# noamzilo/sed-crnn

Hardware: AMD Instinct MI355X
Metric: mel-frames/sec training throughput (seq=256, mel=40) (higher is better)
Workload: dtype f32; 1 GPU; BASELINE config 2: mono (B=128,256,40,1) per GPU, 3xConv3x3(128)+BN+ReLU+pool(1,2)+dropout0.5, BiGRU 2x128, Linear(256,1), BCEWithLogits, Adam lr 1e-3; full fit step (fwd+loss+bwd+allreduce+Adam); global_batch=128, seq_len=256, n_mels=40, parallelism=single

## Files before the change

### include/sedcrnn.h

```cpp
#ifndef SEDCRNN_H
#define SEDCRNN_H

#include <stddef.h>
#include <stdint.h>

#ifdef __cplusplus
extern "C" {
#endif

#define SED_MAX_CONV 4
#define SED_MAX_GRU 4
#define SED_MAX_DENSE 4

int sed_version(void);
const char* sed_last_error_string(void);

int sed_conv3x3_pack_weights(const float* w_oihw, float* wp_fwd, float* wp_dgrad,
                             int Cout, int Cin, void* stream);

int sed_conv3x3_stat_rows(int B, int Cin, int F, int T, int Cout, int x_is_nchw);

int sed_conv3x3_fwd(const float* x, int x_is_nchw, const float* wp, const float* bias,
                    float* y, float* stat_partials,
                    int B, int Cin, int F, int T, int Cout, void* stream);

int sed_conv3x3_pack_weights_ex(const float* w_oihw, float* wp_fwd, float* wp_dgrad, int Cout, int Cin, int mode, void* stream);
int sed_conv3x3_fwd_ex(const float* x, int x_is_nchw, const float* wp, const float* bias, float* y, float* stat_partials,
                       int B, int Cin, int F, int T, int Cout, int mode, void* stream);

size_t sed_conv3x3_wgrad_workspace_bytes(int B, int Cin, int F, int T, int Cout);
int sed_conv3x3_wgrad(const float* x, int x_is_nchw, const float* dy, float* dw_oihw,
                      void* workspace, int B, int Cin, int F, int T, int Cout, void* stream);

#define SED_WGRAD_ZERO_ROW_CLEAN 0x100
#define SED_WGRAD_DIRECT 0x200
size_t sed_conv3x3_wgrad_zero_row_bytes(int B, int Cin, int F, int T, int Cout);
int sed_conv3x3_wgrad_ex(const float* x, int x_is_nchw, const float* dy, float* dw_oihw,
                         void* workspace, int B, int Cin, int F, int T, int Cout, int mode, void* stream);

int sed_conv3x3_bn_relu_pool_eval_supported(int B, int Cin, int F, int T, int Cout);
int sed_conv3x3_pack_weights_bn_folded(const float* w, const float* bias, const float* gamma, const float* beta,
                                       const float* running_mean, const float* running_var, float eps,
                                       float* wf, float* bias_folded, int Cout, int Cin, void* stream);
int sed_conv3x3_bn_relu_pool_eval(const float* x, const float* wp_folded, const float* bias_folded, float* pooled,
                                  int B, int Cin, int F, int T, int Cout, void* stream);
int sed_conv3x3_bf16_eval_supported(int B, int Cin, int F, int T, int Cout);
int sed_conv3x3_bf16_pack_weights_bn_folded(const float* w, const float* bias, const float* gamma, const float* beta,
                                            const float* running_mean, const float* running_var, float eps,
                                            void* wf_bf16, float* bias_folded, int Cout, int Cin, void* stream);
int sed_conv3x3_bf16_bn_relu_pool_eval(const void* x, int x_is_bf16, const void* wf_bf16, const float* bias_folded,
                                       void* pooled_bf16, int B, int Cin, int F, int T, int Cout, void* stream);
int sed_conv3x3_dgrad_bnred_rows(int B, int C, int F, int T, int Cin);
int sed_conv3x3_dgrad_bnred(const float* dy, const float* wp_dgrad, float* dx, float* partials, const float* pooled,
                            const float* gamma, const float* beta, const float* conv_out_below, const float* mean,
                            const float* rstd, float drop_p, int pool_f, int pool_t, int Fy, int Ty,
                            int B, int C, int F, int T, int Cin, void* stream);
int sed_conv3x3_wino_rows(int B, int Cin, int F, int T, int Cout);
int sed_conv3x3_wino_phase_ticks(unsigned long long* buf);
size_t sed_conv3x3_wino_packed_floats(int Cout, int Cin);
int sed_conv3x3_wino_pack_weights(const float* w_oihw, float* uf, float* ud, int Cout, int Cin, void* stream);
int sed_conv3x3_wino_fwd(const float* x, const float* uf, const float* bias, float* y, float* stat_partials,
                         int B, int Cin, int F, int T, int Cout, void* stream);
int sed_conv3x3_wino_dgrad_bnred(const float* dy, const float* ud, float* dx, float* partials, const float* pooled,
                                 const float* gamma, const float* beta, const float* conv_out_below, const float* mean,
                                 const float* rstd, float drop_p, int pool_f, int pool_t, int Fy, int Ty,
                                 int B, int C, int F, int T, int Cin, void* stream);
int sed_conv3x3_wino_pack_weights_bn_folded(const float* w_oihw, const float* bias, const float* gamma, const float* beta,
                                            const float* running_mean, const float* running_var, float eps,
                                            float* uf, float* bias_folded, int Cout, int Cin, void* stream);
int sed_conv3x3_wino_bn_relu_pool_eval(const float* x, const float* uf_folded, const float* bias_folded, float* pooled,
                                       int B, int Cin, int F, int T, int Cout, void* stream);
int sed_conv3x3_wino_rg_rows(int B, int C, int F, int T, int Cin, int Cin1);
int sed_conv3x3_wino_dgrad_bnred_rg(const float* dy, const float* ud, float* dx, float* partials, const float* pooled,
                                    const float* gamma, const float* beta, const float* mean, const float* rstd, float drop_p,
                                    const float* x1, int Cin1, const unsigned char* argmax_bits, float* rg_partials,
                                    int B, int C, int F, int T, int Cin, void* stream);
int sed_conv3x3_dgrad_bnred_rg_rows(int B, int C, int F, int T, int Cin, int Cin1);
int sed_conv3x3_dgrad_bnred_rg(const float* dy, const float* wp_dgrad, float* dx, float* partials, const float* pooled,
                               const float* gamma, const float* beta, const float* mean, const float* rstd, float drop_p,
                               const float* x1, int Cin1, const unsigned char* argmax_bits, float* rg_partials,
                               int B, int C, int F, int T, int Cin, void* stream);

int sed_bn_finalize_train(const float* stat_partials, int rows, int C, double count,
                          const float* gamma, const float* beta,
                          float* running_mean, float* running_var, float momentum, float eps,
                          float* mean, float* rstd, float* scale, float* shift, void* stream);
int sed_bn_stat_sums(const float* stat_partials, int rows, int C, float* sums, void* stream);
int sed_bn_finalize_from_sums(const float* sums, int C, double count, const float* gamma, const float* beta,
                              float* running_mean, float* running_var, float momentum, float eps,
                              float* mean, float* rstd, float* scale, float* shift, void* stream);
int sed_bn_finalize_eval(const float* gamma, const float* beta, const float* running_mean,
                         const float* running_var, float eps, int C,
                         float* scale, float* shift, void* stream);

int sed_bn_relu_pool_drop_fwd(const float* y, const float* scale, const float* shift, float* out,
                              int B, int T, int F, int C, int pool_f, int pool_t, int out_tcf,
                              float drop_p, uint64_t seed, const uint64_t* seed_dev, void* stream);

int sed_bn_relu_pool_route(const float* y, const float* scale, const float* shift, unsigned char* route,
                           int B, int T, int F, int C, int pool_f, int pool_t, void* stream);
int sed_bn_bwd_rows(int B, int T, int pool_t);
int sed_bn_relu_pool_drop_bwd_reduce(const float* y, const float* dout, const float* scale,
                                     const float* shift, const float* mean, const float* rstd,
                                     float* partials, int B, int T, int F, int C, int pool_f,
                                     int pool_t, int out_tcf, float drop_p, uint64_t seed, const uint64_t* seed_dev, void* stream);
int sed_bn_bwd_finalize(const float* partials, int rows, int C, float* sum_g, float* sum_gx,
                        float* dgamma, float* dbeta, void* stream);
int sed_bn_bwd_finalize_small_gamma(const float* partials, int rows, int C, float* sum_g, float* sum_gx,
                                    float* dgamma, float* dbeta, const float* dpooled, const float* pooled,
                                    const float* y, const float* gamma, const float* beta, const float* mean,
                                    const float* rstd, const float* scale, const float* shift,
                                    int B, int T, int F, int pool_f, int pool_t, float drop_p, void* stream);
int sed_bn_bwd_reduce_pooled_supported(int F, int C, int pool_f, int pool_t, int out_tcf);
int sed_bn_bwd_reduce_pooled(const float* pooled, const float* dout, const float* gamma, const float* beta,
                             const float* y, const float* mean, const float* rstd, const float* scale, const float* shift,
                             float* partials, int B, int T, int F, int C, int pool_f, int pool_t, int out_tcf, float drop_p, void* stream);
int sed_bn_relu_pool_drop_bwd_apply(const float* y, const float* dout, const float* scale,
                                    const float* shift, const float* mean, const float* rstd,
                                    const float* sum_g, const float* sum_gx, float* dy,
                                    float* dbias_partials, int B, int T, int F, int C, int pool_f,
                                    int pool_t, int out_tcf, float drop_p, uint64_t seed, const uint64_t* seed_dev, void* stream);
int sed_reduce_rows(const float* partials, int rows, int C, int row_stride, float* out, void* stream);

int sed_conv1_fused_supported(int Cin, int F, int T, int C, int pool_f, int pool_t);
int sed_conv1_fused_rows(int B, int T);
size_t sed_conv1_stats_workspace_bytes(int B, int Cin, int T);
size_t sed_conv1_moments_doubles(int Cin);
int sed_conv1_stats(const float* x, const float* wp, const float* bias, float* stat_partials, void* workspace,
                    int B, int Cin, int F, int T, int C, double* moments, void* stream);
int sed_conv1_bn_relu_pool_drop_fwd(const float* x, const float* wp, const float* bias, const float* scale,
                                    const float* shift, float* out, int B, int Cin, int F, int T, int C,
                                    int pool_f, int pool_t, float drop_p, uint64_t seed, const uint64_t* seed_dev,
                                    unsigned char* argmax_bits, void* stream);
int sed_conv1_route(const float* x, const float* wp, const float* bias, const float* scale, const float* shift,
                    unsigned char* route, int B, int Cin, int F, int T, int C, int pool_f, int pool_t, void* stream);
int sed_conv1_bwd_reduce(const float* x, const float* wp, const float* bias, const float* dout,
                         const float* scale, const float* shift, const float* mean, const float* rstd,
                         float* partials, int B, int Cin, int F, int T, int C, int pool_f, int pool_t,
                         float drop_p, uint64_t seed, const uint64_t* seed_dev, void* stream);
size_t sed_conv1_bwd_apply_workspace_bytes(int B, int Cin, int T, int C);
int sed_conv1_bwd_apply_wgrad(const float* x, const float* wp, const float* bias, const float* dout,
                              const float* scale, const float* shift, const float* mean, const float* rstd,
                              const float* sum_g, const float* sum_gx, float* dw_oihw, float* dbias,
                              void* workspace, int B, int Cin, int F, int T, int C, int pool_f, int pool_t,
                              float drop_p, uint64_t seed, const uint64_t* seed_dev,
                              const float* gamma, const float* beta, float* dgamma, void* stream);

int sed_conv1_rgrad_supported(int Cin, int F, int T, int C, int pool_f, int pool_t);
size_t sed_conv1_bwd_wgrad_workspace_bytes(int B, int Cin, int T, int C);
int sed_conv1_bwd_wgrad(const float* x, const float* dout, const float* pooled, const unsigned char* argmax_bits,
                        const double* moments, const float* wp, const float* bias, const float* mean, const float* rstd,
                        const float* scale, const float* sum_g, const float* sum_gx, float* dw_oihw, float* dbias,
                        void* workspace, int B, int Cin, int F, int T, int C, float drop_p,
                        const float* gamma, const float* beta, float* dgamma, void* stream);
int sed_conv1_bwd_wgrad_assemble(const float* partials, int rows, const double* moments, const float* wp, const float* bias,
                                 const float* mean, const float* rstd, const float* scale, const float* sum_g,
                                 const float* sum_gx, float* dw_oihw, float* dbias, int B, int Cin, int F, int T, int C,
                                 const float* gamma, const float* beta, float* dgamma, void* stream);

int sed_gemm_f32(const float* A, long a_si, long a_sk, const float* B, long b_sk, long b_sj,
                 float* C, long ldc, const float* bias, float beta, int M, int N, int K, void* stream);
size_t sed_gemm_f32_workspace_bytes(int M, int N, int K);
int sed_gemm_f32_ws(const float* A, long a_si, long a_sk, const float* B, long b_sk, long b_sj,
                    float* C, long ldc, const float* bias, int M, int N, int K, void* workspace, void* stream);

int sed_gemm_bf16_nt(const void* A, const void* B, const float* bias, float* C, long ldc, int M, int N, int K, void* stream);

int sed_gemm_f32_wgrad(const float* A, long a_si, long a_sk, const float* B, long b_sk, long b_sj,
                       float* C, long ldc, int M, int N, int K, void* workspace, void* stream);

int sed_linear_fwd(const float* x, const float* W, const float* b, float* y,
                   int M, int K, int N, int relu, void* stream);
size_t sed_linear_bwd_workspace_bytes(int M, int K, int N);
int sed_linear_bwd(const float* x, const float* W, const float* y, float* dy, float* dx,
                   float* dW, float* db, void* workspace, int M, int K, int N, int relu, void* stream);

size_t sed_gru_seq_workspace_bytes(int H);
int sed_gru_seq_fwd(const float* gi, const float* const* whh, const float* const* bhh,
                    float* out, float* saved, void* workspace, int B, int T, int H, void* stream);
size_t sed_gru_seq_bwd_workspace_bytes(int B, int H);
int sed_gru_seq_bwd(const float* dout, const float* saved, const float* const* whh,
                    float* dgi, float* dgh, float* const* dbih, float* const* dbhh, void* workspace,
                    int B, int T, int H, void* stream);
int sed_gru_seq_variant(int B, int H, int* bt, int* hreg, int* hlds);

int sed_loss_fwd_bwd(const float* logits, const float* targets, int n, int kind, float alpha,
                     float gamma, int reduction_mean, float* loss, float* dlogits, float* probs,
                     void* stream);
int sed_sigmoid(const float* x, float* y, int n, void* stream);
int sed_scale(float* x, long n, float alpha, void* stream);

size_t sed_sqnorm_workspace_bytes(long n);
int sed_grad_norm_clip_coef(const float* g, long n, float max_norm, float* norm_out,
                            void* workspace, void* stream);
int sed_adam_step(float* p, const float* g, float* m, float* v, long n, float lr, float beta1,
                  float beta2, float eps, float weight_decay, int step, const float* grad_scale,
                  const uint64_t* step_state, void* stream);
int sed_step_advance(uint64_t* step_state, void* stream);

size_t sed_logmel_tables_bytes(const float* melfb_host, int n_fft, int n_mels);
int sed_logmel_build_tables(const float* window_host, const float* melfb_host, int n_fft, int n_mels,
                            void* tables_host, size_t tables_bytes);
int sed_logmel(const float* pcm, long n_samples, const void* tables, size_t tables_bytes,
               const float* mu, const float* inv_sigma, float* out,
               int n_fft, int hop, int n_mels, int pad_mode, void* stream);
size_t sed_logmel_batch_workspace_bytes(int R);
int sed_logmel_batch(const float* pcm, long pcm_len, const long* clips_host, int R, const void* tables, size_t tables_bytes,
                     const float* mu, const float* inv_sigma, float* out, long out_rows, int n_fft, int hop, int n_mels,
                     int pad_mode, void* workspace, size_t workspace_bytes, void* stream);
size_t sed_logmel_multi_workspace_bytes(int R, int channels);
int sed_logmel_multi(const float* pcm, long pcm_len, const long* clips_host, int R, int channels, const void* tables,
                     size_t tables_bytes, const float* mu, const float* inv_sigma, float* out, long out_rows, int n_fft, int hop,
                     int n_mels, int pad_mode, void* workspace, size_t workspace_bytes, void* stream);
size_t sed_logmel_gcc_workspace_bytes(int R, int channels);
int sed_logmel_gcc(const float* pcm, long pcm_len, const long* clips_host, int R, int channels, const void* tables,
                   size_t tables_bytes, const float* mu, const float* inv_sigma, float* out, long out_rows, int n_fft, int hop,
                   int n_mels, int n_lags, int pad_mode, void* workspace, size_t workspace_bytes, void* stream);
size_t sed_event_tdoa_workspace_bytes(int R, int channels, long E, long max_n_samples, int hop, int max_frames);
int sed_event_tdoa(const float* pcm, long pcm_len, const long* clips_host, int R, int channels, const void* tables,
                   size_t tables_bytes, const int* ev_rec, const int* ev_onset, const int* ev_offset, const int* ev_peak_frame,
                   long E, int time_factor, int hop, int pad_mode, int max_lag, int max_frames, float* lag_out, float* strength_out,
                   int* frames_out, float* acc_out, void* workspace, size_t workspace_bytes, void* stream);

size_t sed_pcen_workspace_bytes(long rows, int R, int W);
int sed_pcen(float* x, long rows, int stride, int col0, int W, const long* recs_host, int R, float* state, double smooth_b,
             float gain, float bias, float power, float eps, float scale, const float* mu, const float* inv_sigma,
             void* workspace, size_t workspace_bytes, void* stream);

size_t sed_resample_workspace_bytes(int R);
int sed_resample_check_table(const long* rows_host, int R, long x_frames, long hist_len, long out_len, int L, int M, int half);
int sed_resample(const void* x, long x_frames, int format, int channels, float* hist, long hist_len, const float* taps,
                 long taps_len, int L, int M, int half, const long* rows_host, int R, float* out, long out_len, void* workspace,
                 size_t workspace_bytes, void* stream);
size_t sed_resample_select_workspace_bytes(int R);
int sed_resample_select_check_table(const long* rows_host, int R, int channels, long x_frames, long hist_len, long out_len, int L,
                                    int M, int half);
int sed_resample_select(const void* x, long x_frames, int format, int channels, float* hist, long hist_len, const float* taps,
                        long taps_len, int L, int M, int half, const long* rows_host, int R, float* out, long out_len,
                        void* workspace, size_t workspace_bytes, void* stream);

int sed_window_batch(const float* mel, const float* lab, long N, int C, int F, int K, const int* starts,
                     const int* tmask, const int* fmask, int n_masks, int time_w, int freq_w,
                     float* x, float* y, int B, int L, int pool, void* stream);
int sed_pack_sequences(const float* feat, long N, int C, int F, int S, int time_last, float* out, void* stream);
size_t sed_col_mean_std_workspace_bytes(int F);
int sed_col_mean_std(const float* x, long N, int F, double* mean, double* stdv, void* workspace, void* stream);
int sed_col_standardize(const float* x, long N, int F, const double* mean, const double* stdv, float* out, void* stream);

#define SED_SEGMENT_COUNTS 17
int sed_segment_counts(const float* pred, const float* lab, long rows, int K, int block, float threshold,
                       unsigned long long* counts17, void* stream);

int sed_detect_stitch(const float* logits, long n_win, int win_out, int K, int hop_out, long last_start_out, long n_out,
                      int combine, int trim, float* probs, void* stream);
size_t sed_detect_workspace_bytes(long n_out, int K, int max_events);
int sed_detect_events(const float* probs, long n_out, int K, int median, float lo, float hi, int min_gap, int min_len,
                      int max_events, void* workspace, size_t workspace_bytes, int* cls, int* onset, int* offset,
                      float* peak, int* peak_frame, int* count, void* stream);
size_t sed_detect_batch_workspace_bytes(long n_total, int K, int R, int max_events);
int sed_detect_stitch_batch(const float* logits, long logits_len, const long* recs_host, int R, int K, int combine, int trim,
                            float* probs, long n_total, void* workspace, size_t workspace_bytes, void* stream);
int sed_detect_events_batch(const float* probs, const long* n_out_host, int R, int K, int median, float lo, float hi, int min_gap,
                            int min_len, int max_events, void* workspace, size_t workspace_bytes, int* rec, int* cls, int* onset,
                            int* offset, float* peak, int* peak_frame, int* event_off, void* stream);

typedef struct sed_tune_setting { int median; float lo, hi; int min_gap, min_len; } sed_tune_setting;
size_t sed_tune_workspace_bytes(long n_total, int K, int R, int n_tracks, int G);
int sed_tune_sweep(const float* probs, const long* n_out_host, int R, int K, const sed_tune_setting* settings_host, int G,
                   const int* ref_off, const int* ref_onset, const int* ref_offset, const int* ref_tol, int collar, int block,
                   void* workspace, size_t workspace_bytes, long* counts, void* stream);

size_t sed_stream_state_bytes(int S, int K, int win_out, int hop_out, int median, int max_new_windows);
int sed_stream_init(void* state, size_t state_bytes, int S, int K, int win_out, int hop_out, int median, int max_new_windows,
                    void* stream);
int sed_stream_reset(void* state, size_t state_bytes, int S, int K, int win_out, int hop_out, int median, int max_new_windows,
                     const int* streams_host, int n_streams, void* stream);
size_t sed_stream_step_workspace_bytes(int S, int K, int max_new_decided);
int sed_stream_step(void* state, size_t state_bytes, int S, int K, int win_out, int hop_out, int median, int max_new_windows,
                    int combine, int trim, float lo, float hi, int min_gap, int min_len, const float* logits, long logits_len,
                    const long* table_host, int max_new_decided, float* probs, long probs_rows, int max_events, int* ev_stream,
                    int* cls, int* onset, int* offset, float* peak, int* peak_frame, int* event_off, void* workspace,
                    size_t workspace_bytes, void* stream);
size_t sed_stream_append_workspace_bytes(int S);
int sed_stream_append(float* buf, long buf_len, long stride, const float* fresh, long fresh_len, float* work, long work_len,
                      const long* table_host, int S, void* workspace, size_t workspace_bytes, void* stream);

typedef sed_tune_setting sed_decoder_setting;
int sed_detect_events_classwise(const float* probs, long n_out, int K, const sed_decoder_setting* classes_host, int max_events,
                                void* workspace, size_t workspace_bytes, int* cls, int* onset, int* offset, float* peak,
                                int* peak_frame, int* count, void* stream);
int sed_detect_events_batch_classwise(const float* probs, const long* n_out_host, int R, int K,
                                      const sed_decoder_setting* classes_host, int max_events, void* workspace, size_t workspace_bytes,
                                      int* rec, int* cls, int* onset, int* offset, float* peak, int* peak_frame, int* event_off,
                                      void* stream);
int sed_stream_step_classwise(void* state, size_t state_bytes, int S, int K, int win_out, int hop_out, int median, int max_new_windows,
                              int combine, int trim, const sed_decoder_setting* classes_host, const float* logits, long logits_len,
                              const long* table_host, int max_new_decided, float* probs, long probs_rows, int max_events,
                              int* ev_stream, int* cls, int* onset, int* offset, float* peak, int* peak_frame, int* event_off,
                              void* workspace, size_t workspace_bytes, void* stream);

typedef struct sed_net_cfg {
    int B, Cin, F, T;
    int n_conv;
    int C[SED_MAX_CONV];
    int pool_f[SED_MAX_CONV], pool_t[SED_MAX_CONV];
    float drop_p[SED_MAX_CONV];
    int n_gru;
    int H[SED_MAX_GRU];
    int n_dense;
    int D[SED_MAX_DENSE];
    float bn_eps, bn_momentum;
    int conv_mode;
    int flags;
} sed_net_cfg;
#define SED_NET_AUX_FIRST 0x1
#define SED_NET_NO_GATE 0x2
#define SED_NET_DIRECT_CONV 0x4

typedef struct sed_net_params {
    float* conv_w[SED_MAX_CONV];
    float* conv_b[SED_MAX_CONV];
    float* bn_g[SED_MAX_CONV];
    float* bn_b[SED_MAX_CONV];
    float* bn_rm[SED_MAX_CONV];
    float* bn_rv[SED_MAX_CONV];
    float* gru_wih[SED_MAX_GRU][2];
    float* gru_whh[SED_MAX_GRU][2];
    float* gru_bih[SED_MAX_GRU][2];
    float* gru_bhh[SED_MAX_GRU][2];
    float* dense_w[SED_MAX_DENSE];
    float* dense_b[SED_MAX_DENSE];
} sed_net_params;

int sed_net_out_shape(const sed_net_cfg* cfg, int* Tp, int* Fp);
size_t sed_net_workspace_bytes(const sed_net_cfg* cfg, int training);
int sed_net_forward(const sed_net_cfg* cfg, const sed_net_params* p, const float* x, float* logits,
                    void* workspace, int training, uint64_t seed, const uint64_t* seed_dev, void* stream);
int sed_net_backward(const sed_net_cfg* cfg, const sed_net_params* p, const sed_net_params* g,
                     const float* x, const float* dlogits, void* workspace, uint64_t seed, const uint64_t* seed_dev,
                     int stage_begin, int stage_end, void* stream, void* aux_stream);
int sed_net_backward_ready_stage(const sed_net_cfg* cfg, int block);

int sed_net_sync_region(const sed_net_cfg* cfg, int backward, int block, size_t* offset_bytes, size_t* n_floats);
int sed_net_forward_phases(const sed_net_cfg* cfg, const sed_net_params* p, const float* x, float* logits,
                           void* workspace, int training, uint64_t seed, int phase_begin, int phase_end,
                           float count_scale, void* stream);
int sed_net_backward_phases(const sed_net_cfg* cfg, const sed_net_params* p, const sed_net_params* g,
                            const float* x, const float* dlogits, void* workspace, uint64_t seed,
                            int phase_begin, int phase_end, float count_scale, void* stream);

int sed_net_workspace_region(const sed_net_cfg* cfg, int training, const char* name, int index,
                             size_t* offset_bytes, size_t* n_floats);

int sed_net_inference_plan(const sed_net_cfg* cfg, int* conv_bf16, int* proj_bf16);

int sed_net_routing(const sed_net_cfg* cfg, const sed_net_params* p, const float* x, const void* workspace, int block,
                    unsigned char* route, void* stream);

enum sed_kernel_tag {
    SED_K_CONV_MFMA_FWD = 0,
    SED_K_CONV_SMALL_FWD,
    SED_K_CONV_MFMA_WGRAD,
    SED_K_CONV_SMALL_WGRAD,
    SED_K_BN_FWD,
    SED_K_BN_BWD_REDUCE,
    SED_K_BN_BWD_APPLY,
    SED_K_GEMM,
    SED_K_GRU_FWD,
    SED_K_GRU_BWD,
    SED_K_ADAM,
    SED_K_LOGMEL,
    SED_K_CONV_MFMA_DGRAD,
    SED_K_COUNT
};
int sed_prof_enable(unsigned tag_mask);
int sed_prof_read(int tag, double* total_ms, long* launches, double* total_units);
const char* sed_prof_tag_name(int tag);
int sed_prof_tag_count(void);

#ifdef __cplusplus
}
#endif
#endif
```

### sed_crnn_amd/_lib.py

```python
import ctypes as C
import os

HERE = os.path.dirname(os.path.abspath(__file__))
LIB_PATH = os.environ.get("SED_CRNN_LIB") or os.path.join(HERE, "libsedcrnn.so")

SED_MAX_CONV = 4
SED_MAX_GRU = 4
SED_MAX_DENSE = 4

_fp = C.c_void_p
_stream = C.c_void_p


class NetCfg(C.Structure):
    _fields_ = [
        ("B", C.c_int), ("Cin", C.c_int), ("F", C.c_int), ("T", C.c_int),
        ("n_conv", C.c_int),
        ("C", C.c_int * SED_MAX_CONV),
        ("pool_f", C.c_int * SED_MAX_CONV), ("pool_t", C.c_int * SED_MAX_CONV),
        ("drop_p", C.c_float * SED_MAX_CONV),
        ("n_gru", C.c_int), ("H", C.c_int * SED_MAX_GRU),
        ("n_dense", C.c_int), ("D", C.c_int * SED_MAX_DENSE),
        ("bn_eps", C.c_float), ("bn_momentum", C.c_float),
        ("conv_mode", C.c_int),
        ("flags", C.c_int),
    ]


class NetParams(C.Structure):
    _fields_ = [
        ("conv_w", _fp * SED_MAX_CONV), ("conv_b", _fp * SED_MAX_CONV),
        ("bn_g", _fp * SED_MAX_CONV), ("bn_b", _fp * SED_MAX_CONV),
        ("bn_rm", _fp * SED_MAX_CONV), ("bn_rv", _fp * SED_MAX_CONV),
        ("gru_wih", (_fp * 2) * SED_MAX_GRU), ("gru_whh", (_fp * 2) * SED_MAX_GRU),
        ("gru_bih", (_fp * 2) * SED_MAX_GRU), ("gru_bhh", (_fp * 2) * SED_MAX_GRU),
        ("dense_w", _fp * SED_MAX_DENSE), ("dense_b", _fp * SED_MAX_DENSE),
    ]


class TuneSetting(C.Structure):
    _fields_ = [("median", C.c_int), ("lo", C.c_float), ("hi", C.c_float), ("min_gap", C.c_int), ("min_len", C.c_int)]


_i, _l, _f, _d, _u64, _sz = C.c_int, C.c_long, C.c_float, C.c_double, C.c_uint64, C.c_size_t
_pp = C.POINTER(_fp)

SIGNATURES = {
    "sed_version": (_i, []),
    "sed_last_error_string": (C.c_char_p, []),
    "sed_conv3x3_pack_weights": (_i, [_fp, _fp, _fp, _i, _i, _stream]),
    "sed_conv3x3_stat_rows": (_i, [_i, _i, _i, _i, _i, _i]),
    "sed_conv3x3_fwd": (_i, [_fp, _i, _fp, _fp, _fp, _fp, _i, _i, _i, _i, _i, _stream]),
    "sed_conv3x3_pack_weights_ex": (_i, [_fp, _fp, _fp, _i, _i, _i, _stream]),
    "sed_conv3x3_fwd_ex": (_i, [_fp, _i, _fp, _fp, _fp, _fp, _i, _i, _i, _i, _i, _i, _stream]),
    "sed_conv3x3_wgrad_workspace_bytes": (_sz, [_i, _i, _i, _i, _i]),
    "sed_conv3x3_wgrad_zero_row_bytes": (_sz, [_i, _i, _i, _i, _i]),
    "sed_conv3x3_wgrad": (_i, [_fp, _i, _fp, _fp, _fp, _i, _i, _i, _i, _i, _stream]),
    "sed_conv3x3_wgrad_ex": (_i, [_fp, _i, _fp, _fp, _fp, _i, _i, _i, _i, _i, _i, _stream]),
    "sed_conv3x3_bn_relu_pool_eval_supported": (_i, [_i, _i, _i, _i, _i]),
    "sed_conv3x3_pack_weights_bn_folded": (_i, [_fp, _fp, _fp, _fp, _fp, _fp, _f, _fp, _fp, _i, _i, _stream]),
    "sed_conv3x3_bn_relu_pool_eval": (_i, [_fp, _fp, _fp, _fp, _i, _i, _i, _i, _i, _stream]),
    "sed_conv3x3_bf16_eval_supported": (_i, [_i, _i, _i, _i, _i]),
    "sed_conv3x3_bf16_pack_weights_bn_folded": (_i, [_fp, _fp, _fp, _fp, _fp, _fp, _f, _fp, _fp, _i, _i, _stream]),
    "sed_conv3x3_bf16_bn_relu_pool_eval": (_i, [_fp, _i, _fp, _fp, _fp, _i, _i, _i, _i, _i, _stream]),
    "sed_conv3x3_dgrad_bnred_rows": (_i, [_i, _i, _i, _i, _i]),
    "sed_conv3x3_dgrad_bnred": (_i, [_fp, _fp, _fp, _fp, _fp, _fp, _fp, _fp, _fp, _fp, _f, _i, _i, _i, _i, _i, _i, _i, _i, _i, _stream]),
    "sed_conv3x3_wino_rows": (_i, [_i, _i, _i, _i, _i]),
    "sed_conv3x3_wino_phase_ticks": (_i, [_fp]),
    "sed_conv3x3_wino_packed_floats": (_sz, [_i, _i]),
    "sed_conv3x3_wino_pack_weights": (_i, [_fp, _fp, _fp, _i, _i, _stream]),
    "sed_conv3x3_wino_fwd": (_i, [_fp, _fp, _fp, _fp, _fp, _i, _i, _i, _i, _i, _stream]),
    "sed_conv3x3_wino_dgrad_bnred": (_i, [_fp, _fp, _fp, _fp, _fp, _fp, _fp, _fp, _fp, _fp, _f, _i, _i, _i, _i, _i, _i, _i, _i, _i, _stream]),
    "sed_conv3x3_wino_pack_weights_bn_folded": (_i, [_fp, _fp, _fp, _fp, _fp, _fp, _f, _fp, _fp, _i, _i, _stream]),
    "sed_conv3x3_wino_bn_relu_pool_eval": (_i, [_fp, _fp, _fp, _fp, _i, _i, _i, _i, _i, _stream]),
    "sed_conv3x3_wino_rg_rows": (_i, [_i, _i, _i, _i, _i, _i]),
    "sed_conv3x3_wino_dgrad_bnred_rg": (_i, [_fp, _fp, _fp, _fp, _fp, _fp, _fp, _fp, _fp, _f, _fp, _i, _fp, _fp, _i, _i, _i, _i, _i, _stream]),
    "sed_conv3x3_dgrad_bnred_rg_rows": (_i, [_i, _i, _i, _i, _i, _i]),
    "sed_conv3x3_dgrad_bnred_rg": (_i, [_fp, _fp, _fp, _fp, _fp, _fp, _fp, _fp, _fp, _f, _fp, _i, _fp, _fp, _i, _i, _i, _i, _i, _stream]),
    "sed_conv1_fused_supported": (_i, [_i, _i, _i, _i, _i, _i]),
    "sed_conv1_fused_rows": (_i, [_i, _i]),
    "sed_conv1_stats_workspace_bytes": (_sz, [_i, _i, _i]),
    "sed_conv1_moments_doubles": (_sz, [_i]),
    "sed_conv1_stats": (_i, [_fp, _fp, _fp, _fp, _fp, _i, _i, _i, _i, _i, _fp, _stream]),
    "sed_conv1_bn_relu_pool_drop_fwd": (_i, [_fp, _fp, _fp, _fp, _fp, _fp, _i, _i, _i, _i, _i, _i, _i, _f, _u64, _fp, _fp, _stream]),
    "sed_conv1_rgrad_supported": (_i, [_i, _i, _i, _i, _i, _i]),
    "sed_conv1_bwd_wgrad_workspace_bytes": (_sz, [_i, _i, _i, _i]),
    "sed_conv1_bwd_wgrad": (_i, [_fp, _fp, _fp, _fp, _fp, _fp, _fp, _fp, _fp, _fp, _fp, _fp, _fp, _fp, _fp, _i, _i, _i, _i, _i, _f, _fp, _fp, _fp, _stream]),
    "sed_conv1_bwd_wgrad_assemble": (_i, [_fp, _i, _fp, _fp, _fp, _fp, _fp, _fp, _fp, _fp, _fp, _fp, _i, _i, _i, _i, _i, _fp, _fp, _fp, _stream]),
    "sed_conv1_route": (_i, [_fp, _fp, _fp, _fp, _fp, _fp, _i, _i, _i, _i, _i, _i, _i, _stream]),
    "sed_conv1_bwd_reduce": (_i, [_fp, _fp, _fp, _fp, _fp, _fp, _fp, _fp, _fp, _i, _i, _i, _i, _i, _i, _i, _f, _u64, _fp, _stream]),
    "sed_conv1_bwd_apply_workspace_bytes": (_sz, [_i, _i, _i, _i]),
    "sed_conv1_bwd_apply_wgrad": (_i, [_fp, _fp, _fp, _fp, _fp, _fp, _fp, _fp, _fp, _fp, _fp, _fp, _fp, _i, _i, _i, _i, _i, _i, _i, _f, _u64, _fp, _fp, _fp, _fp, _stream]),
    "sed_bn_finalize_train": (_i, [_fp, _i, _i, _d, _fp, _fp, _fp, _fp, _f, _f, _fp, _fp, _fp, _fp, _stream]),
    "sed_bn_stat_sums": (_i, [_fp, _i, _i, _fp, _stream]),
    "sed_bn_finalize_from_sums": (_i, [_fp, _i, _d, _fp, _fp, _fp, _fp, _f, _f, _fp, _fp, _fp, _fp, _stream]),
    "sed_bn_finalize_eval": (_i, [_fp, _fp, _fp, _fp, _f, _i, _fp, _fp, _stream]),
    "sed_bn_relu_pool_drop_fwd": (_i, [_fp, _fp, _fp, _fp, _i, _i, _i, _i, _i, _i, _i, _f, _u64, _fp, _stream]),
    "sed_bn_relu_pool_route": (_i, [_fp, _fp, _fp, _fp, _i, _i, _i, _i, _i, _i, _stream]),
    "sed_bn_bwd_rows": (_i, [_i, _i, _i]),
    "sed_bn_relu_pool_drop_bwd_reduce": (_i, [_fp, _fp, _fp, _fp, _fp, _fp, _fp, _i, _i, _i, _i, _i, _i, _i, _f, _u64, _fp, _stream]),
    "sed_bn_bwd_finalize": (_i, [_fp, _i, _i, _fp, _fp, _fp, _fp, _stream]),
    "sed_bn_bwd_finalize_small_gamma": (_i, [_fp, _i, _i, _fp, _fp, _fp, _fp, _fp, _fp, _fp, _fp, _fp, _fp, _fp, _fp, _fp, _i, _i, _i, _i, _i, _f, _stream]),
    "sed_bn_bwd_reduce_pooled_supported": (_i, [_i, _i, _i, _i, _i]),
    "sed_bn_bwd_reduce_pooled": (_i, [_fp, _fp, _fp, _fp, _fp, _fp, _fp, _fp, _fp, _fp, _i, _i, _i, _i, _i, _i, _i, _f, _stream]),
    "sed_bn_relu_pool_drop_bwd_apply": (_i, [_fp, _fp, _fp, _fp, _fp, _fp, _fp, _fp, _fp, _fp, _i, _i, _i, _i, _i, _i, _i, _f, _u64, _fp, _stream]),
    "sed_reduce_rows": (_i, [_fp, _i, _i, _i, _fp, _stream]),
    "sed_gemm_f32": (_i, [_fp, _l, _l, _fp, _l, _l, _fp, _l, _fp, _f, _i, _i, _i, _stream]),
    "sed_gemm_f32_workspace_bytes": (_sz, [_i, _i, _i]),
    "sed_gemm_f32_ws": (_i, [_fp, _l, _l, _fp, _l, _l, _fp, _l, _fp, _i, _i, _i, _fp, _stream]),
    "sed_gemm_bf16_nt": (_i, [_fp, _fp, _fp, _fp, _l, _i, _i, _i, _stream]),
    "sed_gemm_f32_wgrad": (_i, [_fp, _l, _l, _fp, _l, _l, _fp, _l, _i, _i, _i, _fp, _stream]),
    "sed_linear_fwd": (_i, [_fp, _fp, _fp, _fp, _i, _i, _i, _i, _stream]),
    "sed_linear_bwd_workspace_bytes": (_sz, [_i, _i, _i]),
    "sed_linear_bwd": (_i, [_fp, _fp, _fp, _fp, _fp, _fp, _fp, _fp, _i, _i, _i, _i, _stream]),
    "sed_gru_seq_workspace_bytes": (_sz, [_i]),
    "sed_gru_seq_fwd": (_i, [_fp, _pp, _pp, _fp, _fp, _fp, _i, _i, _i, _stream]),
    "sed_gru_seq_bwd_workspace_bytes": (_sz, [_i, _i]),
    "sed_gru_seq_bwd": (_i, [_fp, _fp, _pp, _fp, _fp, _pp, _pp, _fp, _i, _i, _i, _stream]),
    "sed_gru_seq_variant": (_i, [_i, _i, C.POINTER(_i), C.POINTER(_i), C.POINTER(_i)]),
    "sed_loss_fwd_bwd": (_i, [_fp, _fp, _i, _i, _f, _f, _i, _fp, _fp, _fp, _stream]),
    "sed_sigmoid": (_i, [_fp, _fp, _i, _stream]),
    "sed_scale": (_i, [_fp, _l, _f, _stream]),
    "sed_sqnorm_workspace_bytes": (_sz, [_l]),
    "sed_grad_norm_clip_coef": (_i, [_fp, _l, _f, _fp, _fp, _stream]),
    "sed_adam_step": (_i, [_fp, _fp, _fp, _fp, _l, _f, _f, _f, _f, _f, _i, _fp, _fp, _stream]),
    "sed_step_advance": (_i, [_fp, _stream]),
    "sed_logmel_tables_bytes": (_sz, [_fp, _i, _i]),
    "sed_logmel_build_tables": (_i, [_fp, _fp, _i, _i, _fp, _sz]),
    "sed_logmel": (_i, [_fp, _l, _fp, _sz, _fp, _fp, _fp, _i, _i, _i, _i, _stream]),
    "sed_logmel_batch_workspace_bytes": (_sz, [_i]),
    "sed_logmel_batch": (_i, [_fp, _l, _fp, _i, _fp, _sz, _fp, _fp, _fp, _l, _i, _i, _i, _i, _fp, _sz, _stream]),
    "sed_logmel_multi_workspace_bytes": (_sz, [_i, _i]),
    "sed_logmel_multi": (_i, [_fp, _l, _fp, _i, _i, _fp, _sz, _fp, _fp, _fp, _l, _i, _i, _i, _i, _fp, _sz, _stream]),
    "sed_logmel_gcc_workspace_bytes": (_sz, [_i, _i]),
    "sed_logmel_gcc": (_i, [_fp, _l, _fp, _i, _i, _fp, _sz, _fp, _fp, _fp, _l, _i, _i, _i, _i, _i, _fp, _sz, _stream]),
    "sed_event_tdoa_workspace_bytes": (_sz, [_i, _i, _l, _l, _i, _i]),
    "sed_event_tdoa": (_i, [_fp, _l, _fp, _i, _i, _fp, _sz, _fp, _fp, _fp, _fp, _l, _i, _i, _i, _i, _i, _fp, _fp, _fp, _fp, _fp, _sz,
                            _stream]),
    "sed_pcen_workspace_bytes": (_sz, [_l, _i, _i]),
    "sed_pcen": (_i, [_fp, _l, _i, _i, _i, _fp, _i, _fp, _d, _f, _f, _f, _f, _f, _fp, _fp, _fp, _sz, _stream]),
    "sed_resample_workspace_bytes": (_sz, [_i]),
    "sed_resample_check_table": (_i, [_fp, _i, _l, _l, _l, _i, _i, _i]),
    "sed_resample": (_i, [_fp, _l, _i, _i, _fp, _l, _fp, _l, _i, _i, _i, _fp, _i, _fp, _l, _fp, _sz, _stream]),
    "sed_resample_select_workspace_bytes": (_sz, [_i]),
    "sed_resample_select_check_table": (_i, [_fp, _i, _i, _l, _l, _l, _i, _i, _i]),
    "sed_resample_select": (_i, [_fp, _l, _i, _i, _fp, _l, _fp, _l, _i, _i, _i, _fp, _i, _fp, _l, _fp, _sz, _stream]),
    "sed_window_batch": (_i, [_fp, _fp, _l, _i, _i, _i, _fp, _fp, _fp, _i, _i, _i, _fp, _fp, _i, _i, _i, _stream]),
    "sed_pack_sequences": (_i, [_fp, _l, _i, _i, _i, _i, _fp, _stream]),
    "sed_col_mean_std_workspace_bytes": (_sz, [_i]),
    "sed_col_mean_std": (_i, [_fp, _l, _i, _fp, _fp, _fp, _stream]),
    "sed_col_standardize": (_i, [_fp, _l, _i, _fp, _fp, _fp, _stream]),
    "sed_segment_counts": (_i, [_fp, _fp, _l, _i, _i, _f, _fp, _stream]),
    "sed_detect_stitch": (_i, [_fp, _l, _i, _i, _i, _l, _l, _i, _i, _fp, _stream]),
    "sed_detect_workspace_bytes": (_sz, [_l, _i, _i]),
    "sed_detect_events": (_i, [_fp, _l, _i, _i, _f, _f, _i, _i, _i, _fp, _sz, _fp, _fp, _fp, _fp, _fp, _fp, _stream]),
    "sed_detect_batch_workspace_bytes": (_sz, [_l, _i, _i, _i]),
    "sed_detect_stitch_batch": (_i, [_fp, _l, _fp, _i, _i, _i, _i, _fp, _l, _fp, _sz, _stream]),
    "sed_detect_events_batch": (_i, [_fp, _fp, _i, _i, _i, _f, _f, _i, _i, _i, _fp, _sz, _fp, _fp, _fp, _fp, _fp, _fp, _fp, _stream]),
    "sed_tune_workspace_bytes": (_sz, [_l, _i, _i, _i, _i]),
    "sed_tune_sweep": (_i, [_fp, _fp, _i, _i, _fp, _i, _fp, _fp, _fp, _fp, _i, _i, _fp, _sz, _fp, _stream]),
    "sed_stream_state_bytes": (_sz, [_i, _i, _i, _i, _i, _i]),
    "sed_stream_init": (_i, [_fp, _sz, _i, _i, _i, _i, _i, _i, _stream]),
    "sed_stream_reset": (_i, [_fp, _sz, _i, _i, _i, _i, _i, _i, _fp, _i, _stream]),
    "sed_stream_step_workspace_bytes": (_sz, [_i, _i, _i]),
    "sed_stream_step": (_i, [_fp, _sz, _i, _i, _i, _i, _i, _i, _i, _i, _f, _f, _i, _i, _fp, _l, _fp, _i, _fp, _l, _i, _fp, _fp, _fp,
                             _fp, _fp, _fp, _fp, _fp, _sz, _stream]),
    "sed_stream_append_workspace_bytes": (_sz, [_i]),
    "sed_stream_append": (_i, [_fp, _l, _l, _fp, _l, _fp, _l, _fp, _i, _fp, _sz, _stream]),
    "sed_detect_events_classwise": (_i, [_fp, _l, _i, _fp, _i, _fp, _sz, _fp, _fp, _fp, _fp, _fp, _fp, _stream]),
    "sed_detect_events_batch_classwise": (_i, [_fp, _fp, _i, _i, _fp, _i, _fp, _sz, _fp, _fp, _fp, _fp, _fp, _fp, _fp, _stream]),
    "sed_stream_step_classwise": (_i, [_fp, _sz, _i, _i, _i, _i, _i, _i, _i, _i, _fp, _fp, _l, _fp, _i, _fp, _l, _i, _fp, _fp, _fp,
                                       _fp, _fp, _fp, _fp, _fp, _sz, _stream]),
    "sed_prof_enable": (_i, [C.c_uint]),
    "sed_prof_read": (_i, [_i, C.POINTER(_d), C.POINTER(_l), C.POINTER(_d)]),
    "sed_prof_tag_name": (C.c_char_p, [_i]),
    "sed_prof_tag_count": (_i, []),
    "sed_net_out_shape": (_i, [C.POINTER(NetCfg), C.POINTER(_i), C.POINTER(_i)]),
    "sed_net_workspace_bytes": (_sz, [C.POINTER(NetCfg), _i]),
    "sed_net_forward": (_i, [C.POINTER(NetCfg), C.POINTER(NetParams), _fp, _fp, _fp, _i, _u64, _fp, _stream]),
    "sed_net_sync_region": (_i, [C.POINTER(NetCfg), _i, _i, C.POINTER(_sz), C.POINTER(_sz)]),
    "sed_net_workspace_region": (_i, [C.POINTER(NetCfg), _i, C.c_char_p, _i, C.POINTER(_sz), C.POINTER(_sz)]),
    "sed_net_routing": (_i, [C.POINTER(NetCfg), C.POINTER(NetParams), _fp, _fp, _i, _fp, _stream]),
    "sed_net_inference_plan": (_i, [C.POINTER(NetCfg), C.POINTER(C.c_int), C.POINTER(C.c_int)]),
    "sed_net_forward_phases": (_i, [C.POINTER(NetCfg), C.POINTER(NetParams), _fp, _fp, _fp, _i, _u64, _i, _i, _f, _stream]),
    "sed_net_backward_phases": (_i, [C.POINTER(NetCfg), C.POINTER(NetParams), C.POINTER(NetParams), _fp, _fp, _fp, _u64, _i, _i, _f, _stream]),
    "sed_net_backward": (_i, [C.POINTER(NetCfg), C.POINTER(NetParams), C.POINTER(NetParams), _fp, _fp, _fp, _u64, _fp, _i, _i, _stream, _stream]),
    "sed_net_backward_ready_stage": (_i, [C.POINTER(NetCfg), _i]),
}

_lib = None


class SedHipError(RuntimeError):
    pass


def lib():
    global _lib
    if _lib is None:
        if not os.path.exists(LIB_PATH):
            raise SedHipError(
                f"{LIB_PATH} is missing: build it with `python -m sed_crnn_amd.build` "
                "(hipcc --offload-arch=gfx950). sed_crnn_amd has no fallback path.")
        L = C.CDLL(LIB_PATH)
        for name, (res, args) in SIGNATURES.items():
            fn = getattr(L, name)
            fn.restype = res
            fn.argtypes = args
        _lib = L
    return _lib


def check(rc, what=""):
    if rc != 0:
        msg = lib().sed_last_error_string().decode("utf-8", "replace")
        raise SedHipError(f"{what or 'libsedcrnn'} failed (code {rc}): {msg}")


def ptr(t):
    if t is None:
        return None
    return C.c_void_p(t.data_ptr())


def stream_ptr():
    import torch
    return C.c_void_p(torch.cuda.current_stream().cuda_stream)
```

### sed_crnn_amd/csrc/wino.hip

```cpp
#include "common.h"
#include "conv_shared.h"
#include <type_traits>

#define WN_CIN 128
#define WN_NHMAX 14

typedef __attribute__((address_space(1))) const void* sed_gptr_t;
typedef __attribute__((address_space(3))) void* sed_lptr_t;

struct WinoGeo {
    int Fw;
    int ncg, Tw, ntile, nblk, TR, F2, H2, HR, nb8, ncoh, NH;
    float invFw, invF2;
    size_t lds;
    unsigned long long* dbg;
};

__global__ void conv_pack_wino_k(const float* __restrict__ w, float* __restrict__ uf, float* __restrict__ ud, int Cout, int Cin,
                                 const float* __restrict__ bias, const float* __restrict__ gamma, const float* __restrict__ beta,
                                 const float* __restrict__ rm, const float* __restrict__ rv, float eps, float* __restrict__ bias_out) {
    const int i = blockIdx.x * blockDim.x + threadIdx.x;
    if (gamma && i < Cout) {
        const float sc = gamma[i] / sqrtf(rv[i] + eps);
        bias_out[i] = (bias ? bias[i] : 0.f) * sc + (beta[i] - rm[i] * sc);
    }
    wino_pack_one(w, uf, ud, Cout, Cin, i, gamma, rv, eps);
}

extern "C" size_t sed_conv3x3_wino_packed_floats(int Cout, int Cin) { return (size_t)16 * Cout * Cin + WN_ZTAIL; }
extern "C" int sed_conv3x3_wino_pack_weights(const float* w, float* uf, float* ud, int Cout, int Cin, void* stream) {
    SED_REQUIRE(w && (uf || ud) && Cout > 0 && Cin > 0 && Cout % 64 == 0 && Cin % 64 == 0, "conv3x3_wino_pack_weights: bad arguments (channel counts: multiples of 64)");
    conv_pack_wino_k<<<cdiv(Cout * Cin, 256), 256, 0, as_stream(stream)>>>(w, uf, ud, Cout, Cin, nullptr, nullptr, nullptr, nullptr, nullptr, 0.f, nullptr);
    SED_LAUNCH_CHECK("conv_pack_wino");
    return 0;
}
extern "C" int sed_conv3x3_wino_pack_weights_bn_folded(const float* w, const float* bias, const float* gamma, const float* beta,
                                                       const float* running_mean, const float* running_var, float eps,
                                                       float* uf, float* bias_folded, int Cout, int Cin, void* stream) {
    SED_REQUIRE(w && gamma && beta && running_mean && running_var && uf && bias_folded && Cout > 0 && Cin > 0 && Cout % 64 == 0 && Cin % 64 == 0,
                "conv3x3_wino_pack_weights_bn_folded: bad arguments (channel counts: multiples of 64)");
    conv_pack_wino_k<<<cdiv(Cout * Cin, 256), 256, 0, as_stream(stream)>>>(w, uf, nullptr, Cout, Cin, bias, gamma, beta, running_mean, running_var, eps, bias_folded);
    SED_LAUNCH_CHECK("conv_pack_wino (folded)");
    return 0;
}

static bool wino_geo(int B, int Cin, int F, int T, int Cout, WinoGeo* g) {
    if (B <= 0 || Cin != WN_CIN || Cout <= 0 || Cout % 64 != 0 || F < 2 || T < 2 || (F & 1) || (T & 1)) return false;
    if ((size_t)B * T * F * Cin >= ((size_t)1 << 32) || (size_t)T * F * Cout >= ((size_t)1 << 30)) return false;
    if ((size_t)T * F * Cin * sizeof(float) >= ((size_t)1 << 31)) return false;
    g->Tw = T / 2;
    bool ok = false;
    for (int ncg = 1; ncg <= 8 && !ok; ncg *= 2) {
        if ((F / 2) % ncg) break;
        g->ncg = ncg; g->Fw = F / 2 / ncg; g->ntile = g->Fw * g->Tw; g->nblk = cdiv(g->ntile, 64);
        int TR = 0;
        for (int blk = 0; blk < g->nblk; ++blk) {
            const int q1 = blk * 64 + 63 < g->ntile ? blk * 64 + 63 : g->ntile - 1;
            const int n = q1 / g->Fw - (blk * 64) / g->Fw + 1;
            if (n > TR) TR = n;
        }
        g->TR = TR; g->F2 = 2 * g->Fw + 2; g->H2 = g->F2 / 2; g->HR = (2 * TR + 2) * g->F2; g->nb8 = cdiv(g->HR, 8);
        g->NH = cdiv(g->nb8, 4);
        ok = g->NH <= WN_NHMAX;
    }
    if (!ok) return false;
    g->NH = WN_NHMAX;
    g->ncoh = Cout / 64;
    g->invFw = 1.0f / (float)g->Fw; g->invF2 = 1.0f / (float)g->F2;
    size_t fl = (size_t)2 * g->NH * 1024;
    if (fl < 32768 + 512) fl = 32768 + 512;
    g->lds = (fl + 64) * sizeof(float);
    g->dbg = nullptr;
    return g->lds <= 160 * 1024;
}

int sed_internal_wino_rows(int B, int Cin, int F, int T, int Cout) {
    WinoGeo g;
    return wino_geo(B, Cin, F, T, Cout, &g) ? B * g.nblk * g.ncg : 0;
}

__device__ __forceinline__ f32x2 wn_pk_fma(f32x2 a, f32x2 b, f32x2 c) {
    f32x2 d;
    asm("v_pk_fma_f32 %0, %1, %2, %3" : "=v"(d) : "v"(a), "v"(b), "v"(c));
    return d;
}
__device__ __forceinline__ f32x2 wn_pk_add(f32x2 a, f32x2 b) {
    f32x2 d;
    asm("v_pk_add_f32 %0, %1, %2" : "=v"(d) : "v"(a), "v"(b));
    return d;
}
__device__ __forceinline__ f32x2 wn_pk_sub(f32x2 a, f32x2 b) {
    f32x2 d;
    asm("v_pk_add_f32 %0, %1, %2 neg_lo:[0,1] neg_hi:[0,1]" : "=v"(d) : "v"(a), "v"(b));
    return d;
}

template <int NH, bool BNR, int RGC = 0, bool EV = false, int ABL = 0>
__global__ __launch_bounds__(256, 1) void conv3x3_wino_k(
    const float* __restrict__ x, const float* __restrict__ uq, const float* __restrict__ bias,
    float* __restrict__ y, float* __restrict__ stat, int B, int F, int T, int Cout, WinoGeo geo, ConvBnRed br) {
    constexpr int CIN = WN_CIN, NCHUNK = CIN / 32, NSTEP = 4 * NCHUNK;
    constexpr int HBUF = NH * 1024;
    constexpr bool RG = RGC > 0;
    static_assert(!RG || BNR, "the tap sums belong to the BatchNorm-backward epilogue");
    static_assert(!EV || !BNR, "the pooling epilogue belongs to the inference forward");
    extern __shared__ __attribute__((aligned(16))) float smem[];
    const int tid = threadIdx.x, lane = tid & 63, wave = __builtin_amdgcn_readfirstlane(tid >> 6);
    const int r = lane & 31, h = lane >> 5;
    unsigned long long tk0 = 0, tk1 = 0, tk2 = 0;
    if (geo.dbg) tk0 = __builtin_amdgcn_s_memrealtime();

    int blka, coh, b;
    {
        const int bx = blockIdx.x, by = blockIdx.y, nba = geo.nblk * geo.ncg;
        if ((gridDim.y & 7) == 0) {
            const int id = by * (int)gridDim.x + bx, xcd = id & 7, j = id >> 3;
            coh = j % geo.ncoh;
            const int jj = j / geo.ncoh;
            b = xcd + 8 * (jj / nba);
            blka = jj % nba;
        } else {
            coh = bx % geo.ncoh; blka = bx / geo.ncoh; b = by;
        }
    }
    const int blk = blka / geo.ncg, cgp = blka - blk * geo.ncg;
    const int fg0 = 2 * cgp * geo.Fw;
    const int Fw = geo.Fw, F2 = geo.F2, H2 = geo.H2, ntile = geo.ntile;
    const int q0 = blk * 64, ty0 = q0 / Fw;
    const int co0 = coh * 64;

    const int ra = wave == 0 ? 0 : (wave == 2 ? 2 : 1);
    const int rb = wave == 0 ? 2 : (wave == 1 ? 2 : (wave == 2 ? 1 : 3));
    const float sg = wave == 1 ? 1.f : -1.f;

    constexpr unsigned WN_OOB = 0x80000000u;
    const __amdgpu_buffer_rsrc_t xrs = __builtin_amdgcn_make_buffer_rsrc((void*)(x + (size_t)b * T * F * CIN), 0, T * F * CIN * 4, 0x00020000);
    unsigned hp[NH];
    {
        const int Q = lane >> 3, pp = lane & 7;
#pragma unroll
        for (int u = 0; u < NH; ++u) {
            const int P = (u * 4 + wave) * 8 + pp;
            const int tt = sed_fdiv(P, geo.invF2), cx = P - tt * F2;
            const int ff = cx < H2 ? 2 * cx : 2 * (cx - H2) + 1;
            const int t = 2 * ty0 - 1 + tt, f = fg0 + ff - 1;
            const bool in = P < geo.HR && t >= 0 && t < T && f >= 0 && f < F;
            hp[u] = in ? (unsigned)((t * F + f) * CIN + Q * 4) * 4u : WN_OOB;
        }
    }
    auto issue_one = [&](int cc, float* buf, int u) {
        __builtin_amdgcn_raw_ptr_buffer_load_lds(xrs, (sed_lptr_t)(buf + (u * 4 + wave) * 256), 16, (int)hp[u], cc * 128, 0, 0);
    };
    auto issue = [&](int cc, float* buf) {
#pragma unroll
        for (int u = 0; u < NH; ++u) issue_one(cc, buf, u);
    };
    issue(0, smem);
    __builtin_amdgcn_sched_barrier(0);

    int aoff[2][2][4];
#pragma unroll
    for (int mt = 0; mt < 2; ++mt) {
        int q = q0 + mt * 32 + r;
        q = q < ntile ? q : ntile - 1;
        const int ty = sed_fdiv(q, geo.invFw), tf = q - ty * Fw;
#pragma unroll
        for (int s = 0; s < 2; ++s)
#pragma unroll
            for (int c = 0; c < 4; ++c) {
                const int P = (2 * (ty - ty0) + (s ? rb : ra)) * F2 + tf + (c & 1) * H2 + (c >> 1);
                aoff[mt][s][c] = (P >> 3) * 256 + h * 32 + (P & 7) * 4;
            }
    }


    unsigned* rowtab = (unsigned*)(smem + (2 * HBUF > 32768 + 512 ? 2 * HBUF : 32768 + 512));
    unsigned* xofftab = rowtab + 64;
    float* xs = (float*)(xofftab + 64);
    const int XT = 4 * geo.TR + 2;
    if (tid < 64) {
        const int q = q0 + tid;
        const int ty = sed_fdiv(q < ntile ? q : 0, geo.invFw), tf = q - ty * Fw;
        rowtab[tid] = q < ntile ? (unsigned)(((EV ? ty : 2 * ty) * F + fg0 + 2 * tf) * Cout) * 4u : 0xFFFFFFFFu;
        if (RG) xofftab[tid] = (unsigned)((fg0 + 2 * tf) * XT + 4 * (ty - ty0));
    }
    if (RG) {
        const float invXT = 1.0f / (float)XT;
        for (int i = tid; i < (F + 2) * XT; i += 256) {
            const int ff = sed_fdiv(i, invXT), tt = i - ff * XT;
            const int f = ff - 1, t = 4 * ty0 - 1 + tt;
            const bool in = f >= 0 && f < F && t >= 0 && t < br.Ty;
#pragma unroll
            for (int ci = 0; ci < RGC; ++ci)
                xs[ci * (F + 2) * XT + i] = in ? br.x1[(((size_t)b * RGC + ci) * F + f) * br.Ty + t] : 0.f;
        }
    }

    f32x16 acc[4][2][2];
#pragma unroll
    for (int nu = 0; nu < 4; ++nu)
#pragma unroll
        for (int mt = 0; mt < 2; ++mt)
#pragma unroll
            for (int nt = 0; nt < 2; ++nt)
#pragma unroll
                for (int j = 0; j < 16; ++j) acc[nu][mt][nt][j] = 0.f;

    const f32x4* wl = (const f32x4*)uq + (size_t)(coh * 16 + wave * 4) * (NCHUNK * 4 * 2 * 64);
    f32x4 bq[4][2];
    const unsigned lane16 = (unsigned)lane * 16u;
    auto load_b = [&](int nu, int st) {
#pragma unroll
        for (int nt = 0; nt < 2; ++nt)
            bq[nu][nt] = *(const f32x4*)((const char*)(wl + ((nu * NSTEP + st) * 2 + nt) * 64) + lane16);
    };
    static_assert(NH <= 16, "the patch DMA of a slice rides in every fourth slot of its first step");
    f32x2 vp[2][2][4][2];
    f32x4 raw[2][2][4];
    f32x2 up[2][4][2];
    const f32x2 sg2 = {sg, sg};
    auto slot_read = [&](const float* buf, int g, int i) {
        const int mt = i >> 3, s2 = (i >> 2) & 1, c = i & 3;
        raw[mt][s2][c] = *(const f32x4*)(buf + aoff[mt][s2][c] + g * 64);
    };
    auto slot_xform = [&](int k, f32x2 (&v)[2][4][2]) {
        const int mt = k >> 4, q = k & 15, hf = q & 1;
        if (q < 8) {
            const int c = q >> 1;
            const f32x2 da = hf ? __builtin_shufflevector(raw[mt][0][c], raw[mt][0][c], 2, 3) : __builtin_shufflevector(raw[mt][0][c], raw[mt][0][c], 0, 1);
            const f32x2 db = hf ? __builtin_shufflevector(raw[mt][1][c], raw[mt][1][c], 2, 3) : __builtin_shufflevector(raw[mt][1][c], raw[mt][1][c], 0, 1);
            up[mt][c][hf] = wn_pk_fma(sg2, db, da);
        } else {
            const int nu = (q - 8) >> 1;
            if (nu == 0) v[mt][0][hf] = wn_pk_sub(up[mt][0][hf], up[mt][2][hf]);
            else if (nu == 1) v[mt][1][hf] = wn_pk_add(up[mt][1][hf], up[mt][2][hf]);
            else if (nu == 2) v[mt][2][hf] = wn_pk_sub(up[mt][2][hf], up[mt][1][hf]);
            else v[mt][3][hf] = wn_pk_sub(up[mt][1][hf], up[mt][3][hf]);
        }
    };
    constexpr int PF = RGC == 2 ? 2 : 4;
    int rq = 0, c4 = 0, cb = 0;
    const char* qb = nullptr;
    const unsigned char* bitq = nullptr;
    unsigned rstride = 0, cstride = 0;
    unsigned rov[4] = {0, 0, 0, 0};
    f32x4 pqv[PF][BNR ? 4 : 1];
    unsigned btv[PF][RG ? 4 : 1];
    f32x4 q_beta = {0, 0, 0, 0}, gm = {0, 0, 0, 0};
#define WN_EPI_LANE() do { rq = lane >> 3; c4 = (lane & 7) * 4; cb = co0 + nt * 32 + c4; } while (0)
#define WN_EPI_STRIDES() do { rstride = (unsigned)(F * Cout) * 4u; cstride = (unsigned)Cout * 4u; } while (0)
#define WN_EPI_ROWS() do { _Pragma("unroll") for (int k = 0; k < 4; ++k) rov[k] = rowtab[mt * 32 + rq + 8 * k]; } while (0)
    auto epi_setup = [&]() {
        const int mt = wave >> 1, nt = wave & 1;
        WN_EPI_LANE();
        qb = (const char*)(br.pooled + (size_t)b * T * F * Cout + cb);
        bitq = RG ? br.bits + (size_t)b * T * F * (Cout >> 2) + (cb >> 2) : nullptr;
        WN_EPI_STRIDES();
        WN_EPI_ROWS();
    };
    auto prefetch_one = [&](int k, int n, f32x4* pqd, unsigned* btd) {
        if (!BNR) return;
        const unsigned off = rov[k] != 0xFFFFFFFFu ? rov[k] + (n & 1) * rstride + (n >> 1) * cstride : 0u;
        pqd[n] = *(const f32x4*)(qb + off);
        if (RG) btd[n] = bitq[off >> 4];
    };

#pragma unroll
    for (int nu = 0; nu < 4; ++nu) load_b(nu, 0);
    __syncthreads();
#pragma unroll
    for (int i = 0; i < 16; ++i) slot_read(smem, 0, i);
#pragma unroll
    for (int k = 0; k < 32; ++k) slot_xform(k, vp[0]);
    if (geo.dbg) tk1 = __builtin_amdgcn_s_memrealtime();
#pragma unroll
    for (int st = 0; st < (BNR ? NSTEP - 1 : NSTEP); ++st) {
        const int cc = st >> 2, g = st & 3, par = st & 1;
        const bool more = cc + 1 < NCHUNK, nxt = st + 1 < NSTEP;
        const float* nbuf = smem + (((st + 1) >> 2) & 1) * HBUF;
        __builtin_amdgcn_sched_barrier(0);
#pragma unroll
        for (int i = 0; i < 64; ++i) {
            const int nu = i >> 4, j = (i >> 2) & 3, mt = (i >> 1) & 1, nt = i & 1;
            acc[nu][mt][nt] = __builtin_amdgcn_mfma_f32_32x32x2f32(vp[par][mt][nu][j >> 1][j & 1], bq[nu][nt][j], acc[nu][mt][nt], 0, 0, 0);
            if (nxt && !(ABL & 4)) {
                if (i < 16) slot_read(nbuf, (st + 1) & 3, i);
                else if (i < 48 && !(ABL & 1)) slot_xform(i - 16, vp[par ^ 1]);
            }
            if (nxt && (i & 15) == 15 && !(ABL & 2)) load_b(nu, st + 1);
            if (g == 0 && more && !(ABL & 8) && (i & 3) == 1 && (i >> 2) < NH) issue_one(cc + 1, smem + ((cc + 1) & 1) * HBUF, i >> 2);
            __builtin_amdgcn_sched_barrier(0);
        }
        if (nxt && (ABL & 5)) {
#pragma unroll
            for (int a = 0; a < 2; ++a)
#pragma unroll
                for (int c = 0; c < 4; ++c) { vp[par ^ 1][a][c][0] = vp[par][a][c][0]; vp[par ^ 1][a][c][1] = vp[par][a][c][1]; }
        }
        if (g == 2 && more) __syncthreads();
    }
    if (BNR) {
        constexpr int par = (NSTEP - 1) & 1;
        epi_setup();
        __builtin_amdgcn_sched_barrier(0);
#pragma unroll
        for (int i = 0; i < 64; ++i) {
            const int nu = i >> 4, j = (i >> 2) & 3, mt = (i >> 1) & 1, nt = i & 1;
            acc[nu][mt][nt] = __builtin_amdgcn_mfma_f32_32x32x2f32(vp[par][mt][nu][j >> 1][j & 1], bq[nu][nt][j], acc[nu][mt][nt], 0, 0, 0);
            if (i < 4 * (PF == 4 ? 4 : 2)) prefetch_one(i >> 2, i & 3, pqv[i >> 2], btv[i >> 2]);
            else if (i == 16) q_beta = *(const f32x4*)(br.beta + cb);
            else if (i == 17) gm = *(const f32x4*)(br.gamma + cb);
            __builtin_amdgcn_sched_barrier(0);
        }
    }
    __syncthreads();
    if (geo.dbg) tk2 = __builtin_amdgcn_s_memrealtime();

#pragma unroll
    for (int mt = 0; mt < 2; ++mt)
#pragma unroll
        for (int nt = 0; nt < 2; ++nt) {
            if (BNR) {
#pragma unroll
                for (int nu = 0; nu < 4; ++nu) asm volatile("" : "+a"(acc[nu][mt][nt]));
            }
            const f32x16 z0 = acc[0][mt][nt] + acc[1][mt][nt] + acc[2][mt][nt];
            const f32x16 z1 = acc[1][mt][nt] - acc[2][mt][nt] - acc[3][mt][nt];
            float* zb0 = smem + ((((wave * 2 + 0) * 2 + mt) * 2 + nt) << 10);
            float* zb1 = smem + ((((wave * 2 + 1) * 2 + mt) * 2 + nt) << 10);
#pragma unroll
            for (int j = 0; j < 16; ++j) {
                const int row = (j & 3) + 8 * (j >> 2) + 4 * h;
                zb0[row * 32 + r] = z0[j];
                zb1[row * 32 + r] = z1[j];
            }
            if (BNR) __builtin_amdgcn_sched_barrier(0);
        }
    __builtin_amdgcn_sched_barrier(0);
    const int mt = wave >> 1, nt = wave & 1;
    if (!BNR) WN_EPI_LANE();
    f32x4 bv = {0, 0, 0, 0};
    if (bias) bv = *(const f32x4*)(bias + cb);
    char* const yb = (char*)(y + (size_t)b * (EV ? T >> 1 : T) * F * Cout + cb);
    f32x4 q_kr = {0, 0, 0, 0}, q_nb = {0, 0, 0, 0}, a1 = {0, 0, 0, 0}, a2 = {0, 0, 0, 0};
    if (BNR) {
#pragma unroll
        for (int e = 0; e < 4; ++e) {
            const bool zero = gm[e] == 0.f || (br.ybelow != nullptr && fabsf(gm[e]) * 64.f < fabsf(q_beta[e]));
            const float rg = zero ? 0.f : 1.0f / gm[e];
            q_kr[e] = br.keep * rg;
            q_nb[e] = -q_beta[e] * rg;
        }
    }
    if (!BNR) WN_EPI_STRIDES();
    f32x4 R[RG ? 9 * RGC : 1];
#pragma unroll
    for (int k = 0; k < (RG ? 9 * RGC : 1); ++k) R[k] = (f32x4){0, 0, 0, 0};
    if (!BNR) WN_EPI_ROWS();
    unsigned xov[4];
#pragma unroll
    for (int k = 0; k < 4; ++k) xov[k] = RG ? xofftab[mt * 32 + rq + 8 * k] : 0u;
    auto prefetch = [&](int k, f32x4* pqd, unsigned* btd) {
#pragma unroll
        for (int n = 0; n < 4; ++n) prefetch_one(k, n, pqd, btd);
    };
    const bool wr_y = !RG || y != nullptr;

    __syncthreads();
    unsigned long long tkx = 0;
    if (BNR && geo.dbg) tkx = __builtin_amdgcn_s_memrealtime();
#pragma unroll
    for (int k = 0; k < 4; ++k) {
        const int m = rq + 8 * k;
        const unsigned ro = rov[k];
        if (PF == 2 && k >= 1 && k + 1 < 4) prefetch(k + 1, pqv[(k + 1) & 1], btv[(k + 1) & 1]);
        if (ro == 0xFFFFFFFFu) continue;
        const unsigned xo = xov[k];
#pragma unroll
        for (int jj = 0; jj < 2; ++jj) {
            f32x4 z[4];
#pragma unroll
            for (int xi = 0; xi < 4; ++xi) z[xi] = *(const f32x4*)(smem + ((((xi * 2 + jj) * 2 + mt) * 2 + nt) << 10) + m * 32 + c4);
            const f32x4 o[2] = {z[0] + z[1] + z[2] + bv, z[1] - z[2] - z[3] + bv};
            if (EV) {
                f32x4 pl;
#pragma unroll
                for (int e = 0; e < 4; ++e) pl[e] = fmaxf(fmaxf(o[0][e], o[1][e]), 0.f);
                *(f32x4*)(yb + ro + jj * cstride) = pl;
                continue;
            }
#pragma unroll
            for (int i = 0; i < 2; ++i) {
                const unsigned off = ro + i * rstride + jj * cstride;
                const f32x4 v = o[i];
                if (wr_y) *(f32x4*)(yb + off) = v;
                if (BNR) {
                    const f32x4 pq = pqv[k & (PF - 1)][jj * 2 + i];
                    f32x4 g0;
#pragma unroll
                    for (int e = 0; e < 4; ++e) g0[e] = pq[e] > 0.f ? v[e] : 0.f;
                    a1 += g0;
                    a2 += g0 * (pq * q_kr + q_nb);
                    if (RG) {
                        const unsigned bt = btv[k & (PF - 1)][jj * 2 + i];
                        f32x4 g1;
#pragma unroll
                        for (int e = 0; e < 4; ++e) g1[e] = ((bt >> e) & 1u) ? g0[e] : 0.f;
                        const f32x4 gA = g0 - g1;
#pragma unroll
                        for (int ci = 0; ci < RGC; ++ci) {
                            const float* xb = xs + ci * (F + 2) * XT + xo + jj * XT + 2 * i;
#pragma unroll
                            for (int kh = 0; kh < 3; ++kh) {
                                const f32x2 x01 = *(const f32x2*)(xb + kh * XT), x23 = *(const f32x2*)(xb + kh * XT + 2);
                                R[(kh * 3 + 0) * RGC + ci] += gA * x01[0] + g1 * x01[1];
                                R[(kh * 3 + 1) * RGC + ci] += gA * x01[1] + g1 * x23[0];
                                R[(kh * 3 + 2) * RGC + ci] += gA * x23[0] + g1 * x23[1];
                            }
                        }
                    }
                } else {
                    a1 += v;
                    a2 += v * v;
                }
            }
        }
    }
    if (stat && !EV) {
        float* red = smem + 32768;
        if (BNR) { a1 *= br.inv_keep; a2 *= br.inv_keep; }
#pragma unroll
        for (int e = 0; e < 4; ++e) {
#pragma unroll
            for (int o = 8; o < 64; o <<= 1) { a1[e] += __shfl_xor(a1[e], o, 64); a2[e] += __shfl_xor(a2[e], o, 64); }
        }
        if (lane < 8) {
            *(f32x4*)(red + (wave * 2 + 0) * 32 + c4) = a1;
            *(f32x4*)(red + (wave * 2 + 1) * 32 + c4) = a2;
        }
        float* red2 = xs + RGC * (F + 2) * XT;
        if (RG) {
#pragma unroll
            for (int k = 0; k < 9 * RGC; ++k) {
                R[k] *= br.inv_keep;
#pragma unroll
                for (int e = 0; e < 4; ++e) {
#pragma unroll
                    for (int o = 8; o < 64; o <<= 1) R[k][e] += __shfl_xor(R[k][e], o, 64);
                }
                if (lane < 8) *(f32x4*)(red2 + (wave * 9 * RGC + k) * 32 + c4) = R[k];
            }
        }
        __syncthreads();
        const size_t row = (size_t)b * geo.nblk * geo.ncg + blka;
        if (tid < 128) {
            const int which = tid >> 6, c = tid & 63, cn = c >> 5, cr = c & 31;
            const float a = red[((0 * 2 + cn) * 2 + which) * 32 + cr] + red[((1 * 2 + cn) * 2 + which) * 32 + cr];
            stat[row * 2 * Cout + which * Cout + co0 + c] = a;
        }
        if (RG && tid < 64) {
            const int cn = tid >> 5, cr = tid & 31;
            float* o = br.rgp + (row * Cout + co0 + tid) * (1 + 9 * RGC);
            o[0] = red[((0 * 2 + cn) * 2 + 0) * 32 + cr] + red[((1 * 2 + cn) * 2 + 0) * 32 + cr];
#pragma unroll
            for (int k = 0; k < 9 * RGC; ++k)
                o[1 + k] = red2[((0 * 2 + cn) * 9 * RGC + k) * 32 + cr] + red2[((1 * 2 + cn) * 9 * RGC + k) * 32 + cr];
        }
    }
    if (geo.dbg && tid == 0) {
        const unsigned long long tk3 = __builtin_amdgcn_s_memrealtime();
        atomicAdd(geo.dbg + 0, tk1 - tk0);
        atomicAdd(geo.dbg + 1, tk2 - tk1);
        atomicAdd(geo.dbg + 2, tk3 - tk2);
        atomicAdd(geo.dbg + 3, 1ull);
        if (BNR) atomicAdd(geo.dbg + 4, tkx - tk2);
    }
}

#undef WN_EPI_LANE
#undef WN_EPI_STRIDES
#undef WN_EPI_ROWS

template <typename K>
static int wino_set_lds(K kernel, size_t bytes) {
    hipError_t e = hipFuncSetAttribute((const void*)kernel, hipFuncAttributeMaxDynamicSharedMemorySize, (int)bytes);
    if (e != hipSuccess) { sed_set_error("hipFuncSetAttribute(%zu B LDS): %s", bytes, hipGetErrorString(e)); return (int)e; }
    return 0;
}

static unsigned long long* g_wino_dbg = nullptr;
#ifdef WN_ABLATION
static int g_wino_abl = 0;
extern "C" int sed_conv3x3_wino_ablate(int mask) { g_wino_abl = mask; return 0; }
#endif
extern "C" int sed_conv3x3_wino_phase_ticks(unsigned long long* buf) { g_wino_dbg = buf; return 0; }

int sed_internal_wino_launch(const float* x, const float* uq, const float* bias, float* y, float* stat, const ConvBnRed* br,
                             int rgc, int B, int Cin, int F, int T, int Cout, hipStream_t s) {
    WinoGeo g;
    SED_REQUIRE(wino_geo(B, Cin, F, T, Cout, &g), "conv3x3_wino: shape B=%d Cin=%d F=%d T=%d Cout=%d is not supported (sed_conv3x3_wino_rows)", B, Cin, F, T, Cout);
    SED_REQUIRE(rgc >= -1 && rgc <= 2 && (rgc <= 0 || (br && br->x1 && br->bits && br->rgp)) && (rgc >= 0 || (!br && !stat)), "conv3x3_wino: bad epilogue arguments");
    g.dbg = g_wino_dbg;
    if (rgc > 0) {
        g.lds += ((size_t)64 + (size_t)rgc * (F + 2) * (4 * g.TR + 2) + (size_t)4 * 9 * rgc * 32) * sizeof(float);
        SED_REQUIRE(g.lds <= 160 * 1024, "conv3x3_wino: the first block's input patch does not fit the LDS (F=%d)", F);
    }
    const dim3 grid(g.nblk * g.ncg * g.ncoh, B);
    const ConvBnRed none{};
#define WN_LAUNCH(NHv, BNRv, RGv, EVv)                                                                                          \
    do {                                                                                                                           \
        SED_TRY(wino_set_lds((conv3x3_wino_k<NHv, BNRv, RGv, EVv>), g.lds));                                                       \
        conv3x3_wino_k<NHv, BNRv, RGv, EVv><<<grid, 256, g.lds, s>>>(x, uq, bias, y, stat, B, F, T, Cout, g, br ? *br : none);     \
    } while (0)
#ifdef WN_ABLATION
    if (g_wino_abl && rgc == 0 && !br) {
        switch (g_wino_abl) {
            case 1: { SED_TRY(wino_set_lds((conv3x3_wino_k<WN_NHMAX, false, 0, false, 1>), g.lds)); conv3x3_wino_k<WN_NHMAX, false, 0, false, 1><<<grid, 256, g.lds, s>>>(x, uq, bias, y, stat, B, F, T, Cout, g, none); break; }
            case 2: { SED_TRY(wino_set_lds((conv3x3_wino_k<WN_NHMAX, false, 0, false, 2>), g.lds)); conv3x3_wino_k<WN_NHMAX, false, 0, false, 2><<<grid, 256, g.lds, s>>>(x, uq, bias, y, stat, B, F, T, Cout, g, none); break; }
            case 4: { SED_TRY(wino_set_lds((conv3x3_wino_k<WN_NHMAX, false, 0, false, 5>), g.lds)); conv3x3_wino_k<WN_NHMAX, false, 0, false, 5><<<grid, 256, g.lds, s>>>(x, uq, bias, y, stat, B, F, T, Cout, g, none); break; }
            case 8: { SED_TRY(wino_set_lds((conv3x3_wino_k<WN_NHMAX, false, 0, false, 8>), g.lds)); conv3x3_wino_k<WN_NHMAX, false, 0, false, 8><<<grid, 256, g.lds, s>>>(x, uq, bias, y, stat, B, F, T, Cout, g, none); break; }
            default: { SED_TRY(wino_set_lds((conv3x3_wino_k<WN_NHMAX, false, 0, false, 15>), g.lds)); conv3x3_wino_k<WN_NHMAX, false, 0, false, 15><<<grid, 256, g.lds, s>>>(x, uq, bias, y, stat, B, F, T, Cout, g, none); break; }
        }
        SED_LAUNCH_CHECK("conv3x3_wino (ablation)");
        return 0;
    }
#endif
    if (rgc == 1) WN_LAUNCH(WN_NHMAX, true, 1, false);
    else if (rgc == 2) WN_LAUNCH(WN_NHMAX, true, 2, false);
    else if (rgc == -1) WN_LAUNCH(WN_NHMAX, false, 0, true);
    else if (br) WN_LAUNCH(WN_NHMAX, true, 0, false);
    else WN_LAUNCH(WN_NHMAX, false, 0, false);
#undef WN_LAUNCH
    SED_LAUNCH_CHECK("conv3x3_wino");
    return 0;
}

extern "C" int sed_conv3x3_wino_rows(int B, int Cin, int F, int T, int Cout) { return sed_internal_wino_rows(B, Cin, F, T, Cout); }

extern "C" int sed_conv3x3_wino_fwd(const float* x, const float* uq, const float* bias, float* y, float* stat,
                                    int B, int Cin, int F, int T, int Cout, void* stream) {
    SED_REQUIRE(x && uq && y, "conv3x3_wino_fwd: null pointer");
    hipStream_t s = as_stream(stream);
    SedProfScope prof(SED_K_CONV_MFMA_FWD, s, 2.0 * 9.0 * Cin * Cout * (double)B * T * F);
    return sed_internal_wino_launch(x, uq, bias, y, stat, nullptr, 0, B, Cin, F, T, Cout, s);
}

extern "C" int sed_conv3x3_wino_dgrad_bnred(const float* dy, const float* ud, float* dx, float* partials, const float* pooled,
                                            const float* gamma, const float* beta, const float* conv_out_below, const float* mean,
                                            const float* rstd, float drop_p, int pool_f, int pool_t, int Fy, int Ty,
                                            int B, int C, int F, int T, int Cin, void* stream) {
    SED_REQUIRE(dy && ud && dx && partials && pooled && gamma && beta && mean && rstd, "conv3x3_wino_dgrad_bnred: null pointer");
    SED_REQUIRE(drop_p >= 0.f && drop_p < 1.f && pool_f >= 1 && pool_t >= 1, "conv3x3_wino_dgrad_bnred: bad drop_p / pool");
    SED_REQUIRE(Ty / pool_t == T && Fy / pool_f == F, "conv3x3_wino_dgrad_bnred: conv output %dx%d does not pool (%d,%d) to %dx%d", Ty, Fy, pool_f, pool_t, T, F);
    hipStream_t s = as_stream(stream);
    SedProfScope prof(SED_K_CONV_MFMA_DGRAD, s, 2.0 * 9.0 * C * Cin * (double)B * T * F);
    const ConvBnRed br{pooled, gamma, beta, conv_out_below, mean, rstd, 1.f - drop_p, 1.f / (1.f - drop_p), pool_f, pool_t, Fy, Ty,
                       nullptr, nullptr, nullptr, 0.f};
    return sed_internal_wino_launch(dy, ud, nullptr, dx, partials, &br, 0, B, C, F, T, Cin, s);
}

extern "C" int sed_conv3x3_wino_rg_rows(int B, int C, int F, int T, int Cin, int Cin1) {
    WinoGeo g;
    if (Cin1 < 1 || Cin1 > 2 || !wino_geo(B, C, F, T, Cin, &g)) return 0;
    const size_t lds = g.lds + ((size_t)64 + (size_t)Cin1 * (F + 2) * (4 * g.TR + 2) + (size_t)4 * 9 * Cin1 * 32) * sizeof(float);
    return lds <= 160 * 1024 ? B * g.nblk * g.ncg : 0;
}
extern "C" int sed_conv3x3_wino_dgrad_bnred_rg(const float* dy, const float* ud, float* dx, float* partials, const float* pooled,
                                               const float* gamma, const float* beta, const float* mean, const float* rstd, float drop_p,
                                               const float* x1, int Cin1, const unsigned char* argmax_bits, float* rg_partials,
                                               int B, int C, int F, int T, int Cin, void* stream) {
    SED_REQUIRE(dy && ud && partials && pooled && gamma && beta && mean && rstd && x1 && argmax_bits && rg_partials, "conv3x3_wino_dgrad_bnred_rg: null pointer");
    SED_REQUIRE(drop_p >= 0.f && drop_p < 1.f && (Cin1 == 1 || Cin1 == 2), "conv3x3_wino_dgrad_bnred_rg: bad drop_p / input channels");
    hipStream_t s = as_stream(stream);
    SedProfScope prof(SED_K_CONV_MFMA_DGRAD, s, 2.0 * 9.0 * C * Cin * (double)B * T * F);
    const ConvBnRed br{pooled, gamma, beta, nullptr, mean, rstd, 1.f - drop_p, 1.f / (1.f - drop_p), 1, 2, F, 2 * T,
                       x1, argmax_bits, rg_partials, 0.f};
    return sed_internal_wino_launch(dy, ud, nullptr, dx, partials, &br, Cin1, B, C, F, T, Cin, s);
}

extern "C" int sed_conv3x3_wino_bn_relu_pool_eval(const float* x, const float* uf_folded, const float* bias_folded, float* pooled,
                                                  int B, int Cin, int F, int T, int Cout, void* stream) {
    SED_REQUIRE(x && uf_folded && bias_folded && pooled, "conv3x3_wino_bn_relu_pool_eval: null pointer");
    hipStream_t s = as_stream(stream);
    SedProfScope prof(SED_K_CONV_MFMA_FWD, s, 2.0 * 9.0 * Cin * Cout * (double)B * T * F);
    return sed_internal_wino_launch(x, uf_folded, bias_folded, pooled, nullptr, nullptr, -1, B, Cin, F, T, Cout, s);
}
```

Measured before the change: 5.920 million mel-frames/s.

## Make Winograd conv kernel persistent with XCD-aware work runs and cross-item prefetch

Replaces the one-tile-per-block grid of the Winograd conv kernel with a persistent grid sized to the CU count. Each block walks a contiguous run of (batch, block, channel-half) items and keeps batches on the same XCD. While the current item's epilogue runs, it prefetches the next item's input patch, weights and patch offsets. The epilogue exchange buffer is halved and parked in two passes so LDS use shrinks. This adds kernel complexity, register pressure and the risk of load imbalance or lower occupancy.

```diff
diff --git a/include/sedcrnn.h b/include/sedcrnn.h
--- a/include/sedcrnn.h
+++ b/include/sedcrnn.h
@@ -57,6 +57,9 @@
                             int B, int C, int F, int T, int Cin, void* stream);
 int sed_conv3x3_wino_rows(int B, int Cin, int F, int T, int Cout);
 int sed_conv3x3_wino_phase_ticks(unsigned long long* buf);
+int sed_conv3x3_wino_plan(int B, int Cin, int F, int T, int Cout, int ncu, int* grid, int* run);
+int sed_conv3x3_wino_items(int B, int Cin, int F, int T, int Cout, int ncu, int run, int w, int* items, int cap);
+int sed_conv3x3_wino_set_run(int run);
 size_t sed_conv3x3_wino_packed_floats(int Cout, int Cin);
 int sed_conv3x3_wino_pack_weights(const float* w_oihw, float* uf, float* ud, int Cout, int Cin, void* stream);
 int sed_conv3x3_wino_fwd(const float* x, const float* uf, const float* bias, float* y, float* stat_partials,
diff --git a/sed_crnn_amd/_lib.py b/sed_crnn_amd/_lib.py
--- a/sed_crnn_amd/_lib.py
+++ b/sed_crnn_amd/_lib.py
@@ -67,6 +67,9 @@
     "sed_conv3x3_dgrad_bnred": (_i, [_fp, _fp, _fp, _fp, _fp, _fp, _fp, _fp, _fp, _fp, _f, _i, _i, _i, _i, _i, _i, _i, _i, _i, _stream]),
     "sed_conv3x3_wino_rows": (_i, [_i, _i, _i, _i, _i]),
     "sed_conv3x3_wino_phase_ticks": (_i, [_fp]),
+    "sed_conv3x3_wino_plan": (_i, [_i, _i, _i, _i, _i, _i, C.POINTER(C.c_int), C.POINTER(C.c_int)]),
+    "sed_conv3x3_wino_items": (_i, [_i, _i, _i, _i, _i, _i, _i, _i, C.POINTER(C.c_int), _i]),
+    "sed_conv3x3_wino_set_run": (_i, [_i]),
     "sed_conv3x3_wino_packed_floats": (_sz, [_i, _i]),
     "sed_conv3x3_wino_pack_weights": (_i, [_fp, _fp, _fp, _i, _i, _stream]),
     "sed_conv3x3_wino_fwd": (_i, [_fp, _fp, _fp, _fp, _fp, _i, _i, _i, _i, _i, _stream]),
diff --git a/sed_crnn_amd/csrc/wino.hip b/sed_crnn_amd/csrc/wino.hip
--- a/sed_crnn_amd/csrc/wino.hip
+++ b/sed_crnn_amd/csrc/wino.hip
@@ -7,14 +7,38 @@
 
 typedef __attribute__((address_space(1))) const void* sed_gptr_t;
 typedef __attribute__((address_space(3))) void* sed_lptr_t;
+
+struct WinoPlan {
+    int xcd;
+    int n, g;
+    int nba, ncoh;
+};
+__host__ __device__ inline void wino_run(const WinoPlan& p, int w, int* first, int* count) {
+    const int j = p.xcd ? w >> 3 : w;
+    const int base = p.n / p.g, rem = p.n - base * p.g;
+    *first = j * base + (j < rem ? j : rem);
+    *count = base + (j < rem ? 1 : 0);
+}
+__host__ __device__ inline void wino_item(const WinoPlan& p, int w, int idx, int* b, int* blka, int* coh) {
+    const int jj = idx / p.ncoh, s = jj / p.nba;
+    *coh = idx - jj * p.ncoh;
+    *blka = jj - s * p.nba;
+    *b = p.xcd ? (w & 7) + 8 * s : s;
+}
 
 struct WinoGeo {
     int Fw;
     int ncg, Tw, ntile, nblk, TR, F2, H2, HR, nb8, ncoh, NH;
     float invFw, invF2;
     size_t lds;
+    WinoPlan pl;
     unsigned long long* dbg;
 };
+
+#define WN_HBUF (WN_NHMAX * 1024)
+#define WN_EXCH WN_HBUF
+#define WN_RED (WN_EXCH + 16384)
+#define WN_TAB (WN_RED + 512 > 2 * WN_HBUF ? WN_RED + 512 : 2 * WN_HBUF)
 
 __global__ void conv_pack_wino_k(const float* __restrict__ w, float* __restrict__ uf, float* __restrict__ ud, int Cout, int Cin,
                                  const float* __restrict__ bias, const float* __restrict__ gamma, const float* __restrict__ beta,
@@ -67,11 +91,25 @@
     g->NH = WN_NHMAX;
     g->ncoh = Cout / 64;
     g->invFw = 1.0f / (float)g->Fw; g->invF2 = 1.0f / (float)g->F2;
-    size_t fl = (size_t)2 * g->NH * 1024;
-    if (fl < 32768 + 512) fl = 32768 + 512;
-    g->lds = (fl + 64) * sizeof(float);
+    g->lds = ((size_t)WN_TAB + 64) * sizeof(float);
     g->dbg = nullptr;
+    g->pl = WinoPlan{0, 0, 0, 0, 0};
     return g->lds <= 160 * 1024;
+}
+
+static size_t wino_rg_lds(const WinoGeo& g, int F, int rgc) {
+    return ((size_t)64 + (size_t)rgc * (F + 2) * (4 * g.TR + 2) + (size_t)4 * 9 * rgc * 32) * sizeof(float);
+}
+
+static void wino_plan(const WinoGeo& g, int B, int ncu, int force, WinoPlan* p, int* grid, int* run) {
+    p->xcd = (B % 8 == 0) ? 1 : 0;
+    p->nba = g.nblk * g.ncg; p->ncoh = g.ncoh;
+    p->n = (p->xcd ? B / 8 : B) * p->nba * p->ncoh;
+    int cu = p->xcd ? cdiv(ncu, 8) : ncu;
+    if (cu < 1) cu = 1;
+    p->g = force > 0 ? cdiv(p->n, force < p->n ? force : p->n) : (p->n < cu ? p->n : cu);
+    *grid = p->xcd ? 8 * p->g : p->g;
+    *run = cdiv(p->n, p->g);
 }
 
 int sed_internal_wino_rows(int B, int Cin, int F, int T, int Cout) {
@@ -105,58 +143,96 @@
     static_assert(!RG || BNR, "the tap sums belong to the BatchNorm-backward epilogue");
     static_assert(!EV || !BNR, "the pooling epilogue belongs to the inference forward");
     extern __shared__ __attribute__((aligned(16))) float smem[];
-    const int tid = threadIdx.x, lane = tid & 63, wave = __builtin_amdgcn_readfirstlane(tid >> 6);
-    const int r = lane & 31, h = lane >> 5;
+    int tid = threadIdx.x, lane = tid & 63;
+    const int wave = __builtin_amdgcn_readfirstlane(tid >> 6);
+    int r = lane & 31, h = lane >> 5;
     unsigned long long tk0 = 0, tk1 = 0, tk2 = 0;
     if (geo.dbg) tk0 = __builtin_amdgcn_s_memrealtime();
 
+    const int bid = blockIdx.x;
+    int first, count;
+    wino_run(geo.pl, bid, &first, &count);
     int blka, coh, b;
-    {
-        const int bx = blockIdx.x, by = blockIdx.y, nba = geo.nblk * geo.ncg;
-        if ((gridDim.y & 7) == 0) {
-            const int id = by * (int)gridDim.x + bx, xcd = id & 7, j = id >> 3;
-            coh = j % geo.ncoh;
-            const int jj = j / geo.ncoh;
-            b = xcd + 8 * (jj / nba);
-            blka = jj % nba;
-        } else {
-            coh = bx % geo.ncoh; blka = bx / geo.ncoh; b = by;
-        }
-    }
-    const int blk = blka / geo.ncg, cgp = blka - blk * geo.ncg;
-    const int fg0 = 2 * cgp * geo.Fw;
+    wino_item(geo.pl, bid, first, &b, &blka, &coh);
     const int Fw = geo.Fw, F2 = geo.F2, H2 = geo.H2, ntile = geo.ntile;
-    const int q0 = blk * 64, ty0 = q0 / Fw;
-    const int co0 = coh * 64;
 
     const int ra = wave == 0 ? 0 : (wave == 2 ? 2 : 1);
     const int rb = wave == 0 ? 2 : (wave == 1 ? 2 : (wave == 2 ? 1 : 3));
     const float sg = wave == 1 ? 1.f : -1.f;
 
     constexpr unsigned WN_OOB = 0x80000000u;
-    const __amdgpu_buffer_rsrc_t xrs = __builtin_amdgcn_make_buffer_rsrc((void*)(x + (size_t)b * T * F * CIN), 0, T * F * CIN * 4, 0x00020000);
+    auto seq_rsrc = [&](int bb) { return __builtin_amdgcn_make_buffer_rsrc((void*)(x + (size_t)bb * T * F * CIN), 0, T * F * CIN * 4, 0x00020000); };
+    auto patch_off = [&](int ln, int u, int ty0_, int fg0_, bool valid) -> unsigned {
+        const int Q = ln >> 3, pp = ln & 7;
+        const int P = (u * 4 + wave) * 8 + pp;
+        const int tt = sed_fdiv(P, geo.invF2), cx = P - tt * F2;
+        const int ff = cx < H2 ? 2 * cx : 2 * (cx - H2) + 1;
+        const int t = 2 * ty0_ - 1 + tt, f = fg0_ + ff - 1;
+        const bool in = valid & (P < geo.HR) & (t >= 0) & (t < T) & (f >= 0) & (f < F);
+        return in ? (unsigned)((t * F + f) * CIN + Q * 4) * 4u : WN_OOB;
+    };
+    auto block_of = [&](int blka_, int* ty0_, int* fg0_) {
+        const int blk_ = blka_ / geo.ncg;
+        *ty0_ = (blk_ * 64) / Fw;
+        *fg0_ = 2 * (blka_ - blk_ * geo.ncg) * Fw;
+    };
+    __amdgpu_buffer_rsrc_t xrs = seq_rsrc(b);
     unsigned hp[NH];
     {
-        const int Q = lane >> 3, pp = lane & 7;
-#pragma unroll
-        for (int u = 0; u < NH; ++u) {
-            const int P = (u * 4 + wave) * 8 + pp;
-            const int tt = sed_fdiv(P, geo.invF2), cx = P - tt * F2;
-            const int ff = cx < H2 ? 2 * cx : 2 * (cx - H2) + 1;
-            const int t = 2 * ty0 - 1 + tt, f = fg0 + ff - 1;
-            const bool in = P < geo.HR && t >= 0 && t < T && f >= 0 && f < F;
-            hp[u] = in ? (unsigned)((t * F + f) * CIN + Q * 4) * 4u : WN_OOB;
-        }
+        int ty0_, fg0_;
+        block_of(blka, &ty0_, &fg0_);
+#pragma unroll
+        for (int u = 0; u < NH; ++u) hp[u] = patch_off(lane, u, ty0_, fg0_, true);
     }
     auto issue_one = [&](int cc, float* buf, int u) {
         __builtin_amdgcn_raw_ptr_buffer_load_lds(xrs, (sed_lptr_t)(buf + (u * 4 + wave) * 256), 16, (int)hp[u], cc * 128, 0, 0);
     };
-    auto issue = [&](int cc, float* buf) {
-#pragma unroll
-        for (int u = 0; u < NH; ++u) issue_one(cc, buf, u);
-    };
-    issue(0, smem);
+#pragma unroll
+    for (int u = 0; u < NH; ++u) issue_one(0, smem, u);
     __builtin_amdgcn_sched_barrier(0);
+
+    unsigned* rowtab = (unsigned*)(smem + WN_TAB);
+    unsigned* xofftab = rowtab + 64;
+    float* xs = (float*)(xofftab + 64);
+    const int XT = 4 * geo.TR + 2;
+    unsigned lane16 = (unsigned)lane * 16u;
+
+    auto frag_base = [&](int coh_) { return (const f32x4*)uq + (size_t)(coh_ * 16 + wave * 4) * (NCHUNK * 4 * 2 * 64); };
+    const f32x4* wl = frag_base(coh);
+    f32x4 bq[4][2];
+    auto load_b = [&](int nu, int st) {
+#pragma unroll
+        for (int nt = 0; nt < 2; ++nt)
+            bq[nu][nt] = *(const f32x4*)((const char*)(wl + ((nu * NSTEP + st) * 2 + nt) * 64) + lane16);
+    };
+    constexpr bool BQ_EARLY = RGC != 2;
+#pragma unroll
+    for (int nu = 0; nu < 4; ++nu) load_b(nu, 0);
+#pragma unroll
+    for (int nu = 0; nu < 4; ++nu) { asm volatile("" :: "v"(bq[nu][0])); asm volatile("" :: "v"(bq[nu][1])); }
+    __syncthreads();
+
+  for (int it = 0; it < count; ++it) {
+    const int blk = blka / geo.ncg;
+    const int fg0 = 2 * (blka - blk * geo.ncg) * Fw;
+    const int q0 = blk * 64, ty0 = q0 / Fw;
+    const int co0 = coh * 64;
+    const bool has_next = it + 1 < count;
+    int nb, nblka, ncoh, nty0, nfg0;
+    wino_item(geo.pl, bid, first + it + (has_next ? 1 : 0), &nb, &nblka, &ncoh);
+    block_of(nblka, &nty0, &nfg0);
+    const __amdgpu_buffer_rsrc_t nxrs = seq_rsrc(nb);
+    const f32x4* const wln = frag_base(ncoh);
+    auto load_bn = [&](int nu) {
+#pragma unroll
+        for (int nt = 0; nt < 2; ++nt) bq[nu][nt] = *(const f32x4*)((const char*)(wln + (nu * NSTEP * 2 + nt) * 64) + lane16);
+    };
+    asm volatile("" : "+v"(tid));
+    lane = tid & 63; r = lane & 31; h = lane >> 5; lane16 = (unsigned)lane * 16u;
+    if (RGC == 2) {
+#pragma unroll
+        for (int u = 0; u < NH; ++u) hp[u] = patch_off(lane, u, ty0, fg0, true);
+    }
 
     int aoff[2][2][4];
 #pragma unroll
@@ -173,26 +249,23 @@
             }
     }
 
-
-    unsigned* rowtab = (unsigned*)(smem + (2 * HBUF > 32768 + 512 ? 2 * HBUF : 32768 + 512));
-    unsigned* xofftab = rowtab + 64;
-    float* xs = (float*)(xofftab + 64);
-    const int XT = 4 * geo.TR + 2;
-    if (tid < 64) {
-        const int q = q0 + tid;
-        const int ty = sed_fdiv(q < ntile ? q : 0, geo.invFw), tf = q - ty * Fw;
-        rowtab[tid] = q < ntile ? (unsigned)(((EV ? ty : 2 * ty) * F + fg0 + 2 * tf) * Cout) * 4u : 0xFFFFFFFFu;
-        if (RG) xofftab[tid] = (unsigned)((fg0 + 2 * tf) * XT + 4 * (ty - ty0));
-    }
-    if (RG) {
-        const float invXT = 1.0f / (float)XT;
-        for (int i = tid; i < (F + 2) * XT; i += 256) {
-            const int ff = sed_fdiv(i, invXT), tt = i - ff * XT;
-            const int f = ff - 1, t = 4 * ty0 - 1 + tt;
-            const bool in = f >= 0 && f < F && t >= 0 && t < br.Ty;
-#pragma unroll
-            for (int ci = 0; ci < RGC; ++ci)
-                xs[ci * (F + 2) * XT + i] = in ? br.x1[(((size_t)b * RGC + ci) * F + f) * br.Ty + t] : 0.f;
+    if (it == 0 || coh == 0) {
+        if (tid < 64) {
+            const int q = q0 + tid;
+            const int ty = sed_fdiv(q < ntile ? q : 0, geo.invFw), tf = q - ty * Fw;
+            rowtab[tid] = q < ntile ? (unsigned)(((EV ? ty : 2 * ty) * F + fg0 + 2 * tf) * Cout) * 4u : 0xFFFFFFFFu;
+            if (RG) xofftab[tid] = (unsigned)((fg0 + 2 * tf) * XT + 4 * (ty - ty0));
+        }
+        if (RG) {
+            const float invXT = 1.0f / (float)XT;
+            for (int i = tid; i < (F + 2) * XT; i += 256) {
+                const int ff = sed_fdiv(i, invXT), tt = i - ff * XT;
+                const int f = ff - 1, t = 4 * ty0 - 1 + tt;
+                const bool in = f >= 0 && f < F && t >= 0 && t < br.Ty;
+#pragma unroll
+                for (int ci = 0; ci < RGC; ++ci)
+                    xs[ci * (F + 2) * XT + i] = in ? br.x1[(((size_t)b * RGC + ci) * F + f) * br.Ty + t] : 0.f;
+            }
         }
     }
 
@@ -206,14 +279,6 @@
 #pragma unroll
                 for (int j = 0; j < 16; ++j) acc[nu][mt][nt][j] = 0.f;
 
-    const f32x4* wl = (const f32x4*)uq + (size_t)(coh * 16 + wave * 4) * (NCHUNK * 4 * 2 * 64);
-    f32x4 bq[4][2];
-    const unsigned lane16 = (unsigned)lane * 16u;
-    auto load_b = [&](int nu, int st) {
-#pragma unroll
-        for (int nt = 0; nt < 2; ++nt)
-            bq[nu][nt] = *(const f32x4*)((const char*)(wl + ((nu * NSTEP + st) * 2 + nt) * 64) + lane16);
-    };
     static_assert(NH <= 16, "the patch DMA of a slice rides in every fourth slot of its first step");
     f32x2 vp[2][2][4][2];
     f32x4 raw[2][2][4];
@@ -242,31 +307,29 @@
     int rq = 0, c4 = 0, cb = 0;
     const char* qb = nullptr;
     const unsigned char* bitq = nullptr;
-    unsigned rstride = 0, cstride = 0;
+    unsigned rstride = 0, cstride = 0, cb4 = 0;
     unsigned rov[4] = {0, 0, 0, 0};
     f32x4 pqv[PF][BNR ? 4 : 1];
     unsigned btv[PF][RG ? 4 : 1];
     f32x4 q_beta = {0, 0, 0, 0}, gm = {0, 0, 0, 0};
-#define WN_EPI_LANE() do { rq = lane >> 3; c4 = (lane & 7) * 4; cb = co0 + nt * 32 + c4; } while (0)
+#define WN_EPI_LANE() do { rq = lane >> 3; c4 = (lane & 7) * 4; cb = co0 + nt * 32 + c4; cb4 = (unsigned)cb * 4u; } while (0)
 #define WN_EPI_STRIDES() do { rstride = (unsigned)(F * Cout) * 4u; cstride = (unsigned)Cout * 4u; } while (0)
-#define WN_EPI_ROWS() do { _Pragma("unroll") for (int k = 0; k < 4; ++k) rov[k] = rowtab[mt * 32 + rq + 8 * k]; } while (0)
+#define WN_EPI_ROWS() do { _Pragma("unroll") for (int k = 0; k < (RGC == 2 ? 2 : 4); ++k) rov[k] = rowtab[mt * 32 + rq + 8 * k]; } while (0)
     auto epi_setup = [&]() {
         const int mt = wave >> 1, nt = wave & 1;
         WN_EPI_LANE();
-        qb = (const char*)(br.pooled + (size_t)b * T * F * Cout + cb);
-        bitq = RG ? br.bits + (size_t)b * T * F * (Cout >> 2) + (cb >> 2) : nullptr;
+        qb = (const char*)(br.pooled + (size_t)b * T * F * Cout);
+        bitq = RG ? br.bits + (size_t)b * T * F * (Cout >> 2) : nullptr;
         WN_EPI_STRIDES();
         WN_EPI_ROWS();
     };
     auto prefetch_one = [&](int k, int n, f32x4* pqd, unsigned* btd) {
         if (!BNR) return;
-        const unsigned off = rov[k] != 0xFFFFFFFFu ? rov[k] + (n & 1) * rstride + (n >> 1) * cstride : 0u;
+        const unsigned off = (rov[k] != 0xFFFFFFFFu ? rov[k] + (n & 1) * rstride + (n >> 1) * cstride : 0u) + cb4;
         pqd[n] = *(const f32x4*)(qb + off);
         if (RG) btd[n] = bitq[off >> 4];
     };
 
-#pragma unroll
-    for (int nu = 0; nu < 4; ++nu) load_b(nu, 0);
     __syncthreads();
 #pragma unroll
     for (int i = 0; i < 16; ++i) slot_read(smem, 0, i);
@@ -288,7 +351,11 @@
                 else if (i < 48 && !(ABL & 1)) slot_xform(i - 16, vp[par ^ 1]);
             }
             if (nxt && (i & 15) == 15 && !(ABL & 2)) load_b(nu, st + 1);
-            if (g == 0 && more && !(ABL & 8) && (i & 3) == 1 && (i >> 2) < NH) issue_one(cc + 1, smem + ((cc + 1) & 1) * HBUF, i >> 2);
+            if (!nxt && BQ_EARLY && (i & 15) == 15) load_bn(nu);
+            if (g == 0 && !(ABL & 8) && (i & 3) == 1 && (i >> 2) < NH) issue_one(more ? cc + 1 : 0, smem + ((cc + 1) & 1) * HBUF, i >> 2);
+            if (st >= 9 && st <= 11 && i >= 49 && i <= 61 && (i - 49) % 3 == 0 && (st - 9) * 5 + (i - 49) / 3 < NH)
+                hp[(st - 9) * 5 + (i - 49) / 3] = patch_off(lane, (st - 9) * 5 + (i - 49) / 3, nty0, nfg0, has_next);
+            if (st == 11 && i == 62) xrs = nxrs;
             __builtin_amdgcn_sched_barrier(0);
         }
         if (nxt && (ABL & 5)) {
@@ -310,38 +377,41 @@
             if (i < 4 * (PF == 4 ? 4 : 2)) prefetch_one(i >> 2, i & 3, pqv[i >> 2], btv[i >> 2]);
             else if (i == 16) q_beta = *(const f32x4*)(br.beta + cb);
             else if (i == 17) gm = *(const f32x4*)(br.gamma + cb);
+            if (BQ_EARLY && (i & 15) == 15) load_bn(nu);
             __builtin_amdgcn_sched_barrier(0);
         }
     }
     __syncthreads();
     if (geo.dbg) tk2 = __builtin_amdgcn_s_memrealtime();
 
-#pragma unroll
-    for (int mt = 0; mt < 2; ++mt)
-#pragma unroll
-        for (int nt = 0; nt < 2; ++nt) {
-            if (BNR) {
-#pragma unroll
-                for (int nu = 0; nu < 4; ++nu) asm volatile("" : "+a"(acc[nu][mt][nt]));
+    auto park = [&](const int half) {
+#pragma unroll
+        for (int mt = 0; mt < 2; ++mt)
+#pragma unroll
+            for (int nt = 0; nt < 2; ++nt) {
+                if (BNR || half) {
+#pragma unroll
+                    for (int nu = 0; nu < 4; ++nu) asm volatile("" : "+a"(acc[nu][mt][nt]));
+                }
+                float* zb0 = smem + WN_EXCH + ((((wave * 2 + 0) * 2 + mt) * 2 + nt) << 9);
+                float* zb1 = smem + WN_EXCH + ((((wave * 2 + 1) * 2 + mt) * 2 + nt) << 9);
+#pragma unroll
+                for (int j = half * 8; j < half * 8 + 8; ++j) {
+                    const int row = (j & 3) + 8 * ((j >> 2) & 1) + 4 * h;
+                    zb0[row * 32 + r] = acc[0][mt][nt][j] + acc[1][mt][nt][j] + acc[2][mt][nt][j];
+                    zb1[row * 32 + r] = acc[1][mt][nt][j] - acc[2][mt][nt][j] - acc[3][mt][nt][j];
+                    if (half && (j & 1)) __builtin_amdgcn_sched_barrier(0);
+                }
+                if (BNR) __builtin_amdgcn_sched_barrier(0);
             }
-            const f32x16 z0 = acc[0][mt][nt] + acc[1][mt][nt] + acc[2][mt][nt];
-            const f32x16 z1 = acc[1][mt][nt] - acc[2][mt][nt] - acc[3][mt][nt];
-            float* zb0 = smem + ((((wave * 2 + 0) * 2 + mt) * 2 + nt) << 10);
-            float* zb1 = smem + ((((wave * 2 + 1) * 2 + mt) * 2 + nt) << 10);
-#pragma unroll
-            for (int j = 0; j < 16; ++j) {
-                const int row = (j & 3) + 8 * (j >> 2) + 4 * h;
-                zb0[row * 32 + r] = z0[j];
-                zb1[row * 32 + r] = z1[j];
-            }
-            if (BNR) __builtin_amdgcn_sched_barrier(0);
-        }
+    };
+    park(0);
     __builtin_amdgcn_sched_barrier(0);
     const int mt = wave >> 1, nt = wave & 1;
     if (!BNR) WN_EPI_LANE();
     f32x4 bv = {0, 0, 0, 0};
-    if (bias) bv = *(const f32x4*)(bias + cb);
-    char* const yb = (char*)(y + (size_t)b * (EV ? T >> 1 : T) * F * Cout + cb);
+    if (!BNR && bias) bv = *(const f32x4*)(bias + cb);
+    char* const yb = (char*)(y + (size_t)b * (EV ? T >> 1 : T) * F * Cout);
     f32x4 q_kr = {0, 0, 0, 0}, q_nb = {0, 0, 0, 0}, a1 = {0, 0, 0, 0}, a2 = {0, 0, 0, 0};
     if (BNR) {
 #pragma unroll
@@ -357,9 +427,6 @@
 #pragma unroll
     for (int k = 0; k < (RG ? 9 * RGC : 1); ++k) R[k] = (f32x4){0, 0, 0, 0};
     if (!BNR) WN_EPI_ROWS();
-    unsigned xov[4];
-#pragma unroll
-    for (int k = 0; k < 4; ++k) xov[k] = RG ? xofftab[mt * 32 + rq + 8 * k] : 0u;
     auto prefetch = [&](int k, f32x4* pqd, unsigned* btd) {
 #pragma unroll
         for (int n = 0; n < 4; ++n) prefetch_one(k, n, pqd, btd);
@@ -369,29 +436,53 @@
     __syncthreads();
     unsigned long long tkx = 0;
     if (BNR && geo.dbg) tkx = __builtin_amdgcn_s_memrealtime();
+    if (!BNR) asm volatile("" :: "v"(bv));
+    if (BQ_EARLY) {
+#pragma unroll
+        for (int nu = 0; nu < 4; ++nu) { asm volatile("" :: "v"(bq[nu][0])); asm volatile("" :: "v"(bq[nu][1])); }
+    }
+    if (BNR && PF == 4) {
+#pragma unroll
+        for (int k = 0; k < 4; ++k)
+#pragma unroll
+            for (int n = 0; n < 4; ++n) {
+                asm volatile("" :: "v"(pqv[k][n]));
+                if (RG) asm volatile("" :: "v"(btv[k][n]));
+            }
+    }
 #pragma unroll
     for (int k = 0; k < 4; ++k) {
-        const int m = rq + 8 * k;
+        if (k == 2) {
+            __syncthreads();
+            asm volatile("" : "+v"(tid));
+            lane = tid & 63; r = lane & 31; h = lane >> 5;
+            park(1);
+            __syncthreads();
+        }
+        const int m = rq + 8 * (k & 1);
         const unsigned ro = rov[k];
-        if (PF == 2 && k >= 1 && k + 1 < 4) prefetch(k + 1, pqv[(k + 1) & 1], btv[(k + 1) & 1]);
+        if (PF == 2 && k >= 1 && k + 1 < 4) {
+            rov[k + 1] = rowtab[mt * 32 + rq + 8 * (k + 1)];
+            prefetch(k + 1, pqv[(k + 1) & 1], btv[(k + 1) & 1]);
+        }
         if (ro == 0xFFFFFFFFu) continue;
-        const unsigned xo = xov[k];
+        const unsigned xo = RG ? xofftab[mt * 32 + rq + 8 * k] : 0u;
 #pragma unroll
         for (int jj = 0; jj < 2; ++jj) {
             f32x4 z[4];
 #pragma unroll
-            for (int xi = 0; xi < 4; ++xi) z[xi] = *(const f32x4*)(smem + ((((xi * 2 + jj) * 2 + mt) * 2 + nt) << 10) + m * 32 + c4);
+            for (int xi = 0; xi < 4; ++xi) z[xi] = *(const f32x4*)(smem + WN_EXCH + ((((xi * 2 + jj) * 2 + mt) * 2 + nt) << 9) + m * 32 + c4);
             const f32x4 o[2] = {z[0] + z[1] + z[2] + bv, z[1] - z[2] - z[3] + bv};
             if (EV) {
                 f32x4 pl;
 #pragma unroll
                 for (int e = 0; e < 4; ++e) pl[e] = fmaxf(fmaxf(o[0][e], o[1][e]), 0.f);
-                *(f32x4*)(yb + ro + jj * cstride) = pl;
+                *(f32x4*)(yb + (ro + jj * cstride + cb4)) = pl;
                 continue;
             }
 #pragma unroll
             for (int i = 0; i < 2; ++i) {
-                const unsigned off = ro + i * rstride + jj * cstride;
+                const unsigned off = ro + i * rstride + jj * cstride + cb4;
                 const f32x4 v = o[i];
                 if (wr_y) *(f32x4*)(yb + off) = v;
                 if (BNR) {
@@ -426,13 +517,14 @@
             }
         }
     }
+    auto xshfl = [&](float v, int o) { return __builtin_bit_cast(float, __builtin_amdgcn_ds_bpermute((lane ^ o) << 2, __builtin_bit_cast(int, v))); };
     if (stat && !EV) {
-        float* red = smem + 32768;
+        float* red = smem + WN_RED;
         if (BNR) { a1 *= br.inv_keep; a2 *= br.inv_keep; }
 #pragma unroll
         for (int e = 0; e < 4; ++e) {
 #pragma unroll
-            for (int o = 8; o < 64; o <<= 1) { a1[e] += __shfl_xor(a1[e], o, 64); a2[e] += __shfl_xor(a2[e], o, 64); }
+            for (int o = 8; o < 64; o <<= 1) { a1[e] += xshfl(a1[e], o); a2[e] += xshfl(a2[e], o); }
         }
         if (lane < 8) {
             *(f32x4*)(red + (wave * 2 + 0) * 32 + c4) = a1;
@@ -446,7 +538,7 @@
 #pragma unroll
                 for (int e = 0; e < 4; ++e) {
 #pragma unroll
-                    for (int o = 8; o < 64; o <<= 1) R[k][e] += __shfl_xor(R[k][e], o, 64);
+                    for (int o = 8; o < 64; o <<= 1) R[k][e] += xshfl(R[k][e], o);
                 }
                 if (lane < 8) *(f32x4*)(red2 + (wave * 9 * RGC + k) * 32 + c4) = R[k];
             }
@@ -467,14 +559,26 @@
                 o[1 + k] = red2[((0 * 2 + cn) * 9 * RGC + k) * 32 + cr] + red2[((1 * 2 + cn) * 9 * RGC + k) * 32 + cr];
         }
     }
-    if (geo.dbg && tid == 0) {
+    if (geo.dbg) {
         const unsigned long long tk3 = __builtin_amdgcn_s_memrealtime();
-        atomicAdd(geo.dbg + 0, tk1 - tk0);
-        atomicAdd(geo.dbg + 1, tk2 - tk1);
-        atomicAdd(geo.dbg + 2, tk3 - tk2);
-        atomicAdd(geo.dbg + 3, 1ull);
-        if (BNR) atomicAdd(geo.dbg + 4, tkx - tk2);
-    }
+        if (tid == 0) {
+            atomicAdd(geo.dbg + 0, tk1 - tk0);
+            atomicAdd(geo.dbg + 1, tk2 - tk1);
+            atomicAdd(geo.dbg + 2, tk3 - tk2);
+            atomicAdd(geo.dbg + 3, 1ull);
+            if (BNR) atomicAdd(geo.dbg + 4, tkx - tk2);
+        }
+        tk0 = tk3;
+    }
+    b = nb; blka = nblka; coh = ncoh;
+    wl = wln;
+    if (!BQ_EARLY) {
+        lane16 = (unsigned)(tid & 63) * 16u;
+#pragma unroll
+        for (int nu = 0; nu < 4; ++nu) load_b(nu, 0);
+    }
+  }
+    asm volatile("s_waitcnt vmcnt(0)" ::: "memory");
 }
 
 #undef WN_EPI_LANE
@@ -494,18 +598,57 @@
 extern "C" int sed_conv3x3_wino_ablate(int mask) { g_wino_abl = mask; return 0; }
 #endif
 extern "C" int sed_conv3x3_wino_phase_ticks(unsigned long long* buf) { g_wino_dbg = buf; return 0; }
+static int g_wino_run = 0;
+extern "C" int sed_conv3x3_wino_set_run(int run) {
+    SED_REQUIRE(run >= 0, "conv3x3_wino_set_run: run %d", run);
+    g_wino_run = run;
+    return 0;
+}
+
+static int wino_ncu() {
+    constexpr int kMaxDev = 64;
+    static thread_local int n_cu[kMaxDev] = {};
+    int dev = 0;
+    if (hipGetDevice(&dev) != hipSuccess || dev < 0 || dev >= kMaxDev) return 0;
+    if (!n_cu[dev] && hipDeviceGetAttribute(&n_cu[dev], hipDeviceAttributeMultiprocessorCount, dev) != hipSuccess) n_cu[dev] = 0;
+    return n_cu[dev];
+}
+
+extern "C" int sed_conv3x3_wino_plan(int B, int Cin, int F, int T, int Cout, int ncu, int* grid, int* run) {
+    WinoGeo g;
+    SED_REQUIRE(grid && run && ncu > 0, "conv3x3_wino_plan: bad arguments");
+    SED_REQUIRE(wino_geo(B, Cin, F, T, Cout, &g), "conv3x3_wino_plan: shape B=%d Cin=%d F=%d T=%d Cout=%d is not supported", B, Cin, F, T, Cout);
+    wino_plan(g, B, ncu, g_wino_run, &g.pl, grid, run);
+    return 0;
+}
+extern "C" int sed_conv3x3_wino_items(int B, int Cin, int F, int T, int Cout, int ncu, int run, int w, int* items, int cap) {
+    WinoGeo g;
+    int grid = 0, r = 0;
+    if (ncu <= 0 || run < 0 || w < 0 || !items || !wino_geo(B, Cin, F, T, Cout, &g)) return -1;
+    wino_plan(g, B, ncu, run, &g.pl, &grid, &r);
+    if (w >= grid) return -1;
+    int first, count;
+    wino_run(g.pl, w, &first, &count);
+    for (int i = 0; i < count && i < cap; ++i) wino_item(g.pl, w, first + i, &items[3 * i], &items[3 * i + 1], &items[3 * i + 2]);
+    return count;
+}
 
 int sed_internal_wino_launch(const float* x, const float* uq, const float* bias, float* y, float* stat, const ConvBnRed* br,
                              int rgc, int B, int Cin, int F, int T, int Cout, hipStream_t s) {
     WinoGeo g;
     SED_REQUIRE(wino_geo(B, Cin, F, T, Cout, &g), "conv3x3_wino: shape B=%d Cin=%d F=%d T=%d Cout=%d is not supported (sed_conv3x3_wino_rows)", B, Cin, F, T, Cout);
+    SED_REQUIRE(!br || !bias, "conv3x3_wino: the data-gradient epilogues take no bias");
     SED_REQUIRE(rgc >= -1 && rgc <= 2 && (rgc <= 0 || (br && br->x1 && br->bits && br->rgp)) && (rgc >= 0 || (!br && !stat)), "conv3x3_wino: bad epilogue arguments");
     g.dbg = g_wino_dbg;
     if (rgc > 0) {
-        g.lds += ((size_t)64 + (size_t)rgc * (F + 2) * (4 * g.TR + 2) + (size_t)4 * 9 * rgc * 32) * sizeof(float);
+        g.lds += wino_rg_lds(g, F, rgc);
         SED_REQUIRE(g.lds <= 160 * 1024, "conv3x3_wino: the first block's input patch does not fit the LDS (F=%d)", F);
     }
-    const dim3 grid(g.nblk * g.ncg * g.ncoh, B);
+    int ngrid = 0, run = 0;
+    const int ncu = wino_ncu();
+    SED_REQUIRE(ncu > 0, "conv3x3_wino: cannot read the device's CU count");
+    wino_plan(g, B, ncu, g_wino_run, &g.pl, &ngrid, &run);
+    const dim3 grid(ngrid);
     const ConvBnRed none{};
 #define WN_LAUNCH(NHv, BNRv, RGv, EVv)                                                                                          \
     do {                                                                                                                           \
@@ -562,7 +705,7 @@
 extern "C" int sed_conv3x3_wino_rg_rows(int B, int C, int F, int T, int Cin, int Cin1) {
     WinoGeo g;
     if (Cin1 < 1 || Cin1 > 2 || !wino_geo(B, C, F, T, Cin, &g)) return 0;
-    const size_t lds = g.lds + ((size_t)64 + (size_t)Cin1 * (F + 2) * (4 * g.TR + 2) + (size_t)4 * 9 * Cin1 * 32) * sizeof(float);
+    const size_t lds = g.lds + wino_rg_lds(g, F, Cin1);
     return lds <= 160 * 1024 ? B * g.nblk * g.ncg : 0;
 }
 extern "C" int sed_conv3x3_wino_dgrad_bnred_rg(const float* dy, const float* ud, float* dx, float* partials, const float* pooled,
```

Result: no change. 5.962 million mel-frames/s (median of 6 runs) (+0.7%).
